# YyzHarry/imbalanced-regression

Measured on NVIDIA H100. Metric: images/sec, higher is better.
Workload: dtype bf16

## Files before the change

imbalanced-regression_b200/_convlib.py:

```python
from ctypes import c_float, c_int, c_int64, c_size_t, c_void_p

import _lib

P = c_void_p
_I9 = [c_int] * 9

_lib.register({
    "dirb200_conv_prep_weights": (c_int, [P, c_int, c_int, c_int, c_int, c_int, P, P, P]),
    "dirb200_input_to_s2d": (c_int, [P, c_int, c_int, c_int, P, P]),
    "dirb200_conv_fprop": (c_int, [P, P, P] + _I9 + [c_int, P]),
    "dirb200_conv_dgrad": (c_int, [P, P, P] + _I9 + [P]),
    "dirb200_conv_wgrad_workspace_bytes": (c_size_t, _I9 + [c_int]),
    "dirb200_conv_wgrad": (c_int, [P, P, P, P, c_size_t] + _I9 + [c_int, c_int, P]),
    "dirb200_conv_plan": (c_int, _I9 + [c_int, c_int, P]),
    "dirb200_conv_fprop_upsampled": (c_int, [P, P, P] + [c_int] * 7 + [P]),
    "dirb200_conv_wgrad_upsampled_workspace_bytes": (c_size_t, [c_int] * 7),
    "dirb200_conv_wgrad_upsampled": (c_int, [P, P, P, P, c_size_t] + [c_int] * 8 + [P]),
    "dirb200_bn_eval_coeffs": (c_int, [c_int, P, P, c_float, P, P, P, P, P]),
    "dirb200_conv_fprop_bn_stats": (c_int, [P, P, P] + _I9 + [c_int, P, P, P]),
    "dirb200_conv_fprop_affine": (c_int, [P, P, P] + _I9 + [P, P, P, c_int, P]),
    "dirb200_conv_dgrad_bn_moments": (c_int, [P, P, P] + _I9 + [P, P, P, P, P, P]),
    "dirb200_bn_finalize_layout": (c_int, [P, P, c_int64, c_int, P, P, c_float, c_float, P, P, P, P, P, P, P]),
    "dirb200_bn_bwd_coeffs_layout": (c_int, [P, P, c_int64, c_int, P, P, P, P, P, P, P]),
})
```

imbalanced-regression_b200/csrc/conv.cuh:

```cuda
#pragma once
#include "common.cuh"

namespace dirb200 {

struct ConvShape {
  int n, h, w, cin, cout, kh, kw, stride, pad, ho, wo;
};

struct StatLayout {
  int rows, n_tiles, bn, group;
};

int conv_fprop(const __nv_bfloat16* x, const __nv_bfloat16* w, __nv_bfloat16* y, const ConvShape& s, bool stem,
               cudaStream_t st, float* stat_partial = nullptr, StatLayout* layout = nullptr);
struct ConvEpilogue {
  const float* scale;
  const float* shift;
  const __nv_bfloat16* residual;
  bool relu;
};
int conv_fprop_affine(const __nv_bfloat16* x, const __nv_bfloat16* w, __nv_bfloat16* out, const ConvShape& s,
                      const ConvEpilogue& epi, cudaStream_t st);
struct DgradBnMoments {
  const __nv_bfloat16* y;
  const float *scale, *shift;
  float* partial;
  StatLayout* layout;
};
bool conv_dgrad_fuses_bn_moments(const ConvShape& s);
int conv_dgrad(const __nv_bfloat16* dy, const __nv_bfloat16* wt, __nv_bfloat16* dx, const ConvShape& s,
               cudaStream_t st, const DgradBnMoments* bnm = nullptr);
int conv_wgrad_splits(const ConvShape& s);
size_t conv_wgrad_workspace_bytes(const ConvShape& s);
int conv_wgrad_partials(const __nv_bfloat16* x, const __nv_bfloat16* dy, float* partial, const ConvShape& s, bool stem,
                        int* splits_out, cudaStream_t st);
int wgrad_reduce(const float* workspace, int splits, float* dw, const ConvShape& s, bool stem, bool accumulate,
                 cudaStream_t st);
int check_upsampled_conv(int n, int h, int w, int cin, int cout, int ho, int wo, const char* who);
int conv_fprop_upsampled(const __nv_bfloat16* x, const __nv_bfloat16* w_fprop, __nv_bfloat16* y, int n, int h, int w,
                         int cin, int cout, int ho, int wo, cudaStream_t st);
size_t conv_wgrad_upsampled_workspace_bytes(int n, int cin, int cout, int ho, int wo);
int conv_wgrad_partials_upsampled(const __nv_bfloat16* x, const __nv_bfloat16* dy, float* partial, int n, int h, int w,
                                  int cin, int cout, int ho, int wo, int* splits_out, cudaStream_t st);
int conv_wgrad(const __nv_bfloat16* x, const __nv_bfloat16* dy, float* dw, float* workspace, const ConvShape& s,
               bool stem, bool accumulate, cudaStream_t st);
struct WgradReduceDesc {
  const float* partial;
  size_t w_off;
  int splits, cout, cin, kh, kw, stem;
};
int wgrad_reduce_all(const WgradReduceDesc* descs_dev, int nlayers, float* grads, cudaStream_t st);
struct PrepDesc {
  size_t w_off;
  int cout, cin, kh, kw, stem;
  __nv_bfloat16 *wf, *wd;
  FastDiv fd_cin, fd_cout, fd_taps;
};
inline PrepDesc make_prep_desc(size_t w_off, int cout, int cin, int kh, int kw, int stem, __nv_bfloat16* wf,
                               __nv_bfloat16* wd) {
  PrepDesc d{w_off, cout, cin, kh, kw, stem, wf, wd, {}, {}, {}};
  d.fd_cin = make_fastdiv((uint32_t)cin);
  d.fd_cout = make_fastdiv((uint32_t)cout);
  d.fd_taps = make_fastdiv((uint32_t)(kh * kw));
  return d;
}
int conv_plan(const ConvShape& s, bool stem, int op, int* plan);
int prep_weights_all(const float* params, const PrepDesc* descs_dev, int nlayers, cudaStream_t st);
int prep_weights(const float* w, int cout, int cin, int kh, int kw, bool stem, __nv_bfloat16* wf, __nv_bfloat16* wd,
                 cudaStream_t st);
int input_to_s2d(const float* x, int n, int h, int w, __nv_bfloat16* out, cudaStream_t st);

}
```

imbalanced-regression_b200/csrc/conv_api.cu:

```cuda
#include "common.cuh"
#include "conv.cuh"

namespace dirb200 {

__global__ void prep_weights_kernel(const float* __restrict__ w, int cout, int cin, int kh, int kw,
                                    __nv_bfloat16* __restrict__ wf, __nv_bfloat16* __restrict__ wd) {
  const int64_t total = (int64_t)cout * cin * kh * kw;
  for (int64_t i = blockIdx.x * (int64_t)blockDim.x + threadIdx.x; i < total; i += (int64_t)gridDim.x * blockDim.x) {
    int c = (int)(i % cin);
    int64_t t = i / cin;
    int s = (int)(t % kw); t /= kw;
    int r = (int)(t % kh);
    int co = (int)(t / kh);
    const float v = w[(((int64_t)co * cin + c) * kh + r) * kw + s];
    const __nv_bfloat16 b = __float2bfloat16_rn(v);
    wf[i] = b;
    if (wd) wd[(((int64_t)c * kh + r) * kw + s) * cout + co] = b;
  }
}

__global__ void prep_stem_weights_kernel(const float* __restrict__ w, int cout, __nv_bfloat16* __restrict__ wf) {
  const int total = cout * 256;
  for (int i = blockIdx.x * blockDim.x + threadIdx.x; i < total; i += gridDim.x * blockDim.x) {
    const int co = i >> 8, k = i & 255;
    const int rp = k >> 6, sp = (k >> 4) & 3, ph = (k >> 3) & 1, pw = (k >> 2) & 1, c = k & 3;
    const int r = 2 * rp + ph - 1, s = 2 * sp + pw - 1;
    float v = 0.f;
    if (c < 3 && r >= 0 && s >= 0 && r < 7 && s < 7) v = w[((co * 3 + c) * 7 + r) * 7 + s];
    wf[i] = __float2bfloat16_rn(v);
  }
}

__global__ void input_to_s2d_kernel(const float* __restrict__ x, int n, int h, int w, __nv_bfloat16* __restrict__ out) {
  const int h2 = h / 2, w2 = w / 2;
  const int64_t total = (int64_t)n * h2 * w2;
  for (int64_t i = blockIdx.x * (int64_t)blockDim.x + threadIdx.x; i < total; i += (int64_t)gridDim.x * blockDim.x) {
    const int xw = (int)(i % w2);
    const int yh = (int)((i / w2) % h2);
    const int b = (int)(i / ((int64_t)w2 * h2));
    __align__(16) __nv_bfloat16 v[16];
#pragma unroll
    for (int ph = 0; ph < 2; ++ph)
#pragma unroll
      for (int pw = 0; pw < 2; ++pw) {
#pragma unroll
        for (int c = 0; c < 3; ++c)
          v[(ph * 2 + pw) * 4 + c] =
              __float2bfloat16_rn(x[(((int64_t)b * 3 + c) * h + (2 * yh + ph)) * w + (2 * xw + pw)]);
        v[(ph * 2 + pw) * 4 + 3] = __float2bfloat16_rn(0.f);
      }
    uint4* o = reinterpret_cast<uint4*>(out + i * 16);
    o[0] = reinterpret_cast<uint4*>(v)[0];
    o[1] = reinterpret_cast<uint4*>(v)[1];
  }
}

__global__ void wgrad_reduce_kernel(const float* __restrict__ partial, int splits, int cout, int cin, int kh, int kw,
                                    int accumulate, float* __restrict__ dw) {
  const int64_t ktot = (int64_t)kh * kw * cin;
  const int64_t total = ktot * cout;
  const int64_t i = blockIdx.x * (int64_t)blockDim.x + threadIdx.x;
  if (i >= total) return;
  const int co = (int)(i / ktot);
  const int64_t k = i - (int64_t)co * ktot;
  float acc = 0.f;
  for (int sp = 0; sp < splits; ++sp) acc += partial[(int64_t)sp * total + i];
  const int c = (int)(k % cin);
  const int t = (int)(k / cin);
  float* o = dw + ((int64_t)co * cin + c) * (kh * kw) + t;
  *o = accumulate ? *o + acc : acc;
}

__global__ void wgrad_reduce_stem_kernel(const float* __restrict__ partial, int splits, int cout, int accumulate,
                                         float* __restrict__ dw) {
  const int total = 256 * cout;
  for (int i = blockIdx.x * blockDim.x + threadIdx.x; i < total; i += gridDim.x * blockDim.x) {
    const int co = i >> 8, k = i & 255;
    const int rp = k >> 6, sp_ = (k >> 4) & 3, ph = (k >> 3) & 1, pw = (k >> 2) & 1, c = k & 3;
    const int r = 2 * rp + ph - 1, s = 2 * sp_ + pw - 1;
    if (c >= 3 || r < 0 || s < 0) continue;
    float acc = 0.f;
    for (int sp = 0; sp < splits; ++sp) acc += partial[(int64_t)sp * total + i];
    float* o = dw + ((co * 3 + c) * 7 + r) * 7 + s;
    *o = accumulate ? *o + acc : acc;
  }
}

__global__ void __launch_bounds__(256)
wgrad_reduce_all_kernel(const WgradReduceDesc* __restrict__ descs, float* __restrict__ grads) {
  const WgradReduceDesc d = descs[blockIdx.y];
  float* dw = grads + d.w_off;
  if (d.stem) {
    const int total = 256 * d.cout;
    for (int i = blockIdx.x * blockDim.x + threadIdx.x; i < total; i += gridDim.x * blockDim.x) {
      const int co = i >> 8, k = i & 255;
      const int rp = k >> 6, sp_ = (k >> 4) & 3, ph = (k >> 3) & 1, pw = (k >> 2) & 1, c = k & 3;
      const int r = 2 * rp + ph - 1, s = 2 * sp_ + pw - 1;
      if (c >= 3 || r < 0 || s < 0) continue;
      float acc = 0.f;
      for (int sp = 0; sp < d.splits; ++sp) acc += d.partial[(int64_t)sp * total + i];
      dw[((co * 3 + c) * 7 + r) * 7 + s] += acc;
    }
    return;
  }
  const int64_t ktot = (int64_t)d.kh * d.kw * d.cin;
  const int64_t total = ktot * d.cout;
  const int taps = d.kh * d.kw;
  for (int64_t i = blockIdx.x * (int64_t)blockDim.x + threadIdx.x; i < total; i += (int64_t)gridDim.x * blockDim.x) {
    const float* p = d.partial + i;
    float a0 = 0.f, a1 = 0.f, a2 = 0.f, a3 = 0.f;
    int sp = 0;
    for (; sp + 4 <= d.splits; sp += 4) {
      a0 += p[(int64_t)sp * total];
      a1 += p[(int64_t)(sp + 1) * total];
      a2 += p[(int64_t)(sp + 2) * total];
      a3 += p[(int64_t)(sp + 3) * total];
    }
    for (; sp < d.splits; ++sp) a0 += p[(int64_t)sp * total];
    const int64_t co = i / ktot, k = i - co * ktot;
    const int c = (int)(k % d.cin), t = (int)(k / d.cin);
    dw[(co * d.cin + c) * taps + t] += (a0 + a1) + (a2 + a3);
  }
}

int wgrad_reduce_all(const WgradReduceDesc* descs_dev, int nlayers, float* grads, cudaStream_t st) {
  if (nlayers <= 0) return DIRB200_OK;
  wgrad_reduce_all_kernel<<<dim3(2 * num_sms(), nlayers), 256, 0, st>>>(descs_dev, grads);
  DIRB_LAUNCHED();
  return DIRB200_OK;
}

__global__ void prep_weights_all_kernel(const float* __restrict__ params, const PrepDesc* __restrict__ descs) {
  const PrepDesc d = descs[blockIdx.y];
  const float* w = params + d.w_off;
  if (d.stem) {
    const int total = d.cout * 256;
    for (int i = blockIdx.x * blockDim.x + threadIdx.x; i < total; i += gridDim.x * blockDim.x) {
      const int co = i >> 8, k = i & 255;
      const int rp = k >> 6, sp = (k >> 4) & 3, ph = (k >> 3) & 1, pw = (k >> 2) & 1, c = k & 3;
      const int r = 2 * rp + ph - 1, s = 2 * sp + pw - 1;
      float v = 0.f;
      if (c < 3 && r >= 0 && s >= 0 && r < 7 && s < 7) v = w[((co * 3 + c) * 7 + r) * 7 + s];
      d.wf[i] = __float2bfloat16_rn(v);
    }
    return;
  }
  const uint32_t taps = (uint32_t)(d.kh * d.kw);
  const uint32_t total = (uint32_t)d.cout * (uint32_t)d.cin * taps;
  const uint32_t stride = gridDim.x * blockDim.x;
  for (uint32_t i = blockIdx.x * blockDim.x + threadIdx.x; i < total; i += stride) {
    uint32_t t, c, co, tap;
    d.fd_cin.divmod(i, t, c);
    d.fd_taps.divmod(t, co, tap);
    d.wf[i] = __float2bfloat16_rn(w[((size_t)co * d.cin + c) * taps + tap]);
  }
  if (!d.wd) return;
  for (uint32_t i = blockIdx.x * blockDim.x + threadIdx.x; i < total; i += stride) {
    uint32_t t, c, co, tap;
    d.fd_cout.divmod(i, t, co);
    d.fd_taps.divmod(t, c, tap);
    d.wd[i] = __float2bfloat16_rn(w[((size_t)co * d.cin + c) * taps + tap]);
  }
}

int prep_weights_all(const float* params, const PrepDesc* descs_dev, int nlayers, cudaStream_t st) {
  prep_weights_all_kernel<<<dim3(96, nlayers), 256, 0, st>>>(params, descs_dev);
  DIRB_LAUNCHED();
  return DIRB200_OK;
}

static inline int grid1d(int64_t n, int block = 256) {
  int64_t g = (n + block - 1) / block;
  const int64_t cap = 8 * (int64_t)num_sms();
  return (int)(g < 1 ? 1 : (g > cap ? cap : g));
}

int prep_weights(const float* w, int cout, int cin, int kh, int kw, bool stem, __nv_bfloat16* wf, __nv_bfloat16* wd,
                 cudaStream_t st) {
  if (stem) {
    prep_stem_weights_kernel<<<grid1d((int64_t)cout * 256), 256, 0, st>>>(w, cout, wf);
  } else {
    prep_weights_kernel<<<grid1d((int64_t)cout * cin * kh * kw), 256, 0, st>>>(w, cout, cin, kh, kw, wf, wd);
  }
  DIRB_LAUNCHED();
  return DIRB200_OK;
}

int input_to_s2d(const float* x, int n, int h, int w, __nv_bfloat16* out, cudaStream_t st) {
  input_to_s2d_kernel<<<grid1d((int64_t)n * (h / 2) * (w / 2)), 256, 0, st>>>(x, n, h, w, out);
  DIRB_LAUNCHED();
  return DIRB200_OK;
}

int wgrad_reduce(const float* workspace, int splits, float* dw, const ConvShape& s, bool stem, bool accumulate,
                 cudaStream_t st) {
  if (stem)
    wgrad_reduce_stem_kernel<<<grid1d(256 * (int64_t)s.cout), 256, 0, st>>>(workspace, splits, s.cout, accumulate, dw);
  else
  {
    const int64_t total = (int64_t)s.kh * s.kw * s.cin * s.cout;
    wgrad_reduce_kernel<<<(unsigned)((total + 255) / 256), 256, 0, st>>>(workspace, splits, s.cout, s.cin, s.kh, s.kw,
                                                                         accumulate, dw);
  }
  DIRB_LAUNCHED();
  return DIRB200_OK;
}

int conv_wgrad(const __nv_bfloat16* x, const __nv_bfloat16* dy, float* dw, float* workspace, const ConvShape& s,
               bool stem, bool accumulate, cudaStream_t st) {
  int splits = 1;
  if (int rc = conv_wgrad_partials(x, dy, workspace, s, stem, &splits, st)) return rc;
  return wgrad_reduce(workspace, splits, dw, s, stem, accumulate, st);
}

static int to_shape(int n, int h, int w, int cin, int cout, int kh, int kw, int stride, int pad, int stem,
                    ConvShape* s) {
  if (stem) {
    DIRB_CHECK_ARG(cin == 3 && kh == 7 && kw == 7 && stride == 2 && pad == 3 && h % 2 == 0 && w % 2 == 0,
                   "stem conv must be 3->Cout 7x7 stride 2 pad 3 on even H, W");
    *s = ConvShape{n, h / 2, w / 2, 16, cout, 4, 4, 1, 2, h / 2, w / 2};
  } else {
    DIRB_CHECK_ARG(n > 0 && h > 0 && w > 0 && kh > 0 && kw > 0 && stride > 0 && pad >= 0, "bad conv shape");
    *s = ConvShape{n, h, w, cin, cout, kh, kw, stride, pad, (h + 2 * pad - kh) / stride + 1,
                   (w + 2 * pad - kw) / stride + 1};
  }
  return DIRB200_OK;
}

}

using namespace dirb200;

extern "C" {

int dirb200_conv_prep_weights(const float* w, int cout, int cin, int kh, int kw, int stem, void* w_fprop,
                              void* w_dgrad, void* stream) {
  DIRB_CHECK_ARG(w && w_fprop && cout > 0 && cin > 0, "conv_prep_weights: bad arguments");
  DIRB_CHECK_ARG(!stem || (cin == 3 && kh == 7 && kw == 7), "conv_prep_weights: stem must be 3x7x7");
  return prep_weights(w, cout, cin, kh, kw, stem != 0, (__nv_bfloat16*)w_fprop, (__nv_bfloat16*)w_dgrad,
                      as_stream(stream));
}

int dirb200_input_to_s2d(const float* x_nchw, int n, int h, int w, void* out_bf16, void* stream) {
  DIRB_CHECK_ARG(x_nchw && out_bf16 && n > 0 && h > 0 && w > 0 && h % 2 == 0 && w % 2 == 0,
                 "input_to_s2d: bad arguments");
  return input_to_s2d(x_nchw, n, h, w, (__nv_bfloat16*)out_bf16, as_stream(stream));
}

int dirb200_conv_fprop(const void* x, const void* w_fprop, void* y, int n, int h, int w, int cin, int cout, int kh,
                       int kw, int stride, int pad, int stem, void* stream) {
  DIRB_CHECK_ARG(x && w_fprop && y, "conv_fprop: null pointer");
  ConvShape s;
  if (int rc = to_shape(n, h, w, cin, cout, kh, kw, stride, pad, stem, &s)) return rc;
  return conv_fprop((const __nv_bfloat16*)x, (const __nv_bfloat16*)w_fprop, (__nv_bfloat16*)y, s, stem != 0,
                    as_stream(stream));
}

int dirb200_conv_dgrad(const void* dy, const void* w_dgrad, void* dx, int n, int h, int w, int cin, int cout, int kh,
                       int kw, int stride, int pad, void* stream) {
  DIRB_CHECK_ARG(dy && w_dgrad && dx, "conv_dgrad: null pointer");
  ConvShape s;
  if (int rc = to_shape(n, h, w, cin, cout, kh, kw, stride, pad, 0, &s)) return rc;
  return conv_dgrad((const __nv_bfloat16*)dy, (const __nv_bfloat16*)w_dgrad, (__nv_bfloat16*)dx, s,
                    as_stream(stream));
}

size_t dirb200_conv_wgrad_workspace_bytes(int n, int h, int w, int cin, int cout, int kh, int kw, int stride, int pad,
                                          int stem) {
  ConvShape s;
  if (to_shape(n, h, w, cin, cout, kh, kw, stride, pad, stem, &s)) return 0;
  return conv_wgrad_workspace_bytes(s);
}

int dirb200_conv_wgrad(const void* x, const void* dy, float* dw, void* workspace, size_t workspace_bytes, int n, int h,
                       int w, int cin, int cout, int kh, int kw, int stride, int pad, int stem, int accumulate,
                       void* stream) {
  DIRB_CHECK_ARG(x && dy && dw && workspace, "conv_wgrad: null pointer");
  ConvShape s;
  if (int rc = to_shape(n, h, w, cin, cout, kh, kw, stride, pad, stem, &s)) return rc;
  if (workspace_bytes < conv_wgrad_workspace_bytes(s)) {
    set_error("conv_wgrad: workspace too small (%zu < %zu)", workspace_bytes, conv_wgrad_workspace_bytes(s));
    return DIRB200_ERR_WORKSPACE;
  }
  return conv_wgrad((const __nv_bfloat16*)x, (const __nv_bfloat16*)dy, dw, (float*)workspace, s, stem != 0,
                    accumulate != 0, as_stream(stream));
}

int dirb200_conv_fprop_upsampled(const void* x, const void* w_fprop, void* y, int n, int h, int w, int cin, int cout,
                                 int ho, int wo, void* stream) {
  DIRB_CHECK_ARG(x && w_fprop && y, "conv_fprop_upsampled: null pointer");
  return conv_fprop_upsampled((const __nv_bfloat16*)x, (const __nv_bfloat16*)w_fprop, (__nv_bfloat16*)y, n, h, w, cin,
                              cout, ho, wo, as_stream(stream));
}

size_t dirb200_conv_wgrad_upsampled_workspace_bytes(int n, int h, int w, int cin, int cout, int ho, int wo) {
  if (check_upsampled_conv(n, h, w, cin, cout, ho, wo, "conv_wgrad_upsampled_workspace_bytes")) return 0;
  return conv_wgrad_upsampled_workspace_bytes(n, cin, cout, ho, wo);
}

int dirb200_conv_wgrad_upsampled(const void* x, const void* dy, float* dw, void* workspace, size_t workspace_bytes, int n,
                                 int h, int w, int cin, int cout, int ho, int wo, int accumulate, void* stream) {
  DIRB_CHECK_ARG(x && dy && dw && workspace, "conv_wgrad_upsampled: null pointer");
  if (int rc = check_upsampled_conv(n, h, w, cin, cout, ho, wo, "conv_wgrad_upsampled")) return rc;
  const size_t need = conv_wgrad_upsampled_workspace_bytes(n, cin, cout, ho, wo);
  if (workspace_bytes < need) {
    set_error("conv_wgrad_upsampled: workspace too small (%zu < %zu)", workspace_bytes, need);
    return DIRB200_ERR_WORKSPACE;
  }
  cudaStream_t st = as_stream(stream);
  int splits = 1;
  if (int rc = conv_wgrad_partials_upsampled((const __nv_bfloat16*)x, (const __nv_bfloat16*)dy, (float*)workspace, n, h,
                                             w, cin, cout, ho, wo, &splits, st))
    return rc;
  const ConvShape s{n, ho, wo, cin, cout, 5, 5, 1, 2, ho, wo};
  return wgrad_reduce((const float*)workspace, splits, dw, s, false, accumulate != 0, st);
}

static void layout_to_host(const StatLayout& l, int* layout_host) {
  layout_host[0] = l.rows; layout_host[1] = l.n_tiles; layout_host[2] = l.bn; layout_host[3] = l.group;
}

int dirb200_conv_fprop_bn_stats(const void* x, const void* w_fprop, void* y, int n, int h, int w, int cin, int cout,
                                int kh, int kw, int stride, int pad, int stem, float* partial, int* layout_host,
                                void* stream) {
  DIRB_CHECK_ARG(x && w_fprop && y && partial && layout_host, "conv_fprop_bn_stats: null pointer");
  ConvShape s;
  if (int rc = to_shape(n, h, w, cin, cout, kh, kw, stride, pad, stem, &s)) return rc;
  StatLayout lay{};
  if (int rc = conv_fprop((const __nv_bfloat16*)x, (const __nv_bfloat16*)w_fprop, (__nv_bfloat16*)y, s, stem != 0,
                          as_stream(stream), partial, &lay))
    return rc;
  layout_to_host(lay, layout_host);
  return DIRB200_OK;
}

int dirb200_conv_fprop_affine(const void* x, const void* w_fprop, void* out, int n, int h, int w, int cin, int cout,
                              int kh, int kw, int stride, int pad, const float* scale, const float* shift,
                              const void* residual, int relu, void* stream) {
  DIRB_CHECK_ARG(x && w_fprop && out, "conv_fprop_affine: null pointer");
  ConvShape s;
  if (int rc = to_shape(n, h, w, cin, cout, kh, kw, stride, pad, 0, &s)) return rc;
  return conv_fprop_affine((const __nv_bfloat16*)x, (const __nv_bfloat16*)w_fprop, (__nv_bfloat16*)out, s,
                           ConvEpilogue{scale, shift, (const __nv_bfloat16*)residual, relu != 0}, as_stream(stream));
}

int dirb200_conv_dgrad_bn_moments(const void* dy, const void* w_dgrad, void* dx, int n, int h, int w, int cin, int cout,
                                  int kh, int kw, int stride, int pad, const void* y_prev, const float* scale,
                                  const float* shift, float* partial, int* layout_host, void* stream) {
  DIRB_CHECK_ARG(dy && w_dgrad && dx && y_prev && scale && shift && partial && layout_host,
                 "conv_dgrad_bn_moments: null pointer");
  ConvShape s;
  if (int rc = to_shape(n, h, w, cin, cout, kh, kw, stride, pad, 0, &s)) return rc;
  StatLayout lay{};
  const DgradBnMoments bm{(const __nv_bfloat16*)y_prev, scale, shift, partial, &lay};
  if (int rc = conv_dgrad((const __nv_bfloat16*)dy, (const __nv_bfloat16*)w_dgrad, (__nv_bfloat16*)dx, s,
                          as_stream(stream), &bm))
    return rc;
  layout_to_host(lay, layout_host);
  return DIRB200_OK;
}

int dirb200_conv_plan(int n, int h, int w, int cin, int cout, int kh, int kw, int stride, int pad, int stem, int op,
                      int* plan7) {
  DIRB_CHECK_ARG(plan7 && op >= 0 && op <= 2, "conv_plan: bad arguments");
  ConvShape s;
  if (int rc = to_shape(n, h, w, cin, cout, kh, kw, stride, pad, stem, &s)) return rc;
  return conv_plan(s, stem != 0, op, plan7);
}

}
```

imbalanced-regression_b200/csrc/conv_igemm.cu:

```cuda
#include <stdlib.h>
#include "common.cuh"
#include "tc.cuh"
#include "conv.cuh"
#include "upsample.cuh"

namespace dirb200 {
using namespace tc;

constexpr int BM = 128;
constexpr int BK = 64;
constexpr int kProducerThreads = 128;
constexpr int kThreads = 384;
constexpr int kMaxTaps = 25;
constexpr int kMaxSmemBytes = 232448;

struct IgemmParams {
  const __nv_bfloat16* src;
  int n, hs, ws, cs;
  int hm, wm;
  int kh, kw, stride, pad;
  int transposed;
  int cls_on, cls_py, cls_px, full_h, full_w;
  int ntaps_c;
  int tap_list[kMaxTaps];
  long long tap_eoff[kMaxTaps];
  unsigned short tap_r[kMaxTaps], tap_s[kMaxTaps];
  FastDiv fd_hw, fd_wm, fd_cpb, fd_kw, fd_ntiles, fd_persplit;
  int cpb;
  long long pixels;
  int num_kblocks;
  int kblocks_per_split;
  int total_chunks;
  int m_tiles, n_tiles;
  int num_tiles;
  int a_mode;
  int i2c_stride, i2c_lo;
  int ldc;
  void* out;
  float* stat_out;
  const float* epi_scale;
  const float* epi_shift;
  const __nv_bfloat16* epi_res;
  int epi_relu;
  const __nv_bfloat16* bst_y;
  const float* bst_scale;
  const float* bst_shift;
  int up_h, up_w;
  float up_sh, up_sw;
};

template <int BN, bool STAGED_EPI>
struct Cfg {
  static constexpr int kABytes = BM * BK * 2;
  static constexpr int kBBytes = BN * BK * 2;
  static constexpr int kStageBytes = kABytes + kBBytes;
  static constexpr int kStages = BN == 128 ? (STAGED_EPI ? 5 : 6) : 8;
  static constexpr int kBarOffset = kStages * kStageBytes;
  static constexpr int kStageRowBytes = BN * 2 + 16;
  static constexpr int kEpiWarpBytes = 16 * kStageRowBytes;
  static constexpr int kEpiOffset = kBarOffset + 256;
  static constexpr int kStatWarpBytes = 2 * BN * 4;
  static constexpr int kStatOffset = kEpiOffset + (STAGED_EPI ? 8 * kEpiWarpBytes : 0);
  static constexpr int kSmemBytes = kStatOffset + (STAGED_EPI ? 8 * kStatWarpBytes : 0) + 1024;
  static_assert(kSmemBytes <= kMaxSmemBytes, "shared memory budget");
};

__device__ __forceinline__ uint32_t pack_pixel(long long p, const IgemmParams& P) {
  if (p >= P.pixels) return 0u;
  uint32_t n, rem, y, x;
  P.fd_hw.divmod(static_cast<uint32_t>(p), n, rem);
  P.fd_wm.divmod(rem, y, x);
  return 0x80000000u | (n << 18) | (y << 9) | x;
}

struct RowPre {
  int nb, yb, xb;
};
__device__ __forceinline__ RowPre row_pre(const IgemmParams& P, uint32_t pk) {
  RowPre rp;
  const int n = (pk >> 18) & 0x1FFF;
  int y = (pk >> 9) & 0x1FF, x = pk & 0x1FF;
  if (P.cls_on) {
    y = 2 * y + P.cls_py;
    x = 2 * x + P.cls_px;
  }
  rp.nb = n * P.hs;
  if (!P.transposed) {
    rp.yb = y * P.stride - P.pad;
    rp.xb = x * P.stride - P.pad;
  } else {
    rp.yb = y + P.pad;
    rp.xb = x + P.pad;
  }
  if (!(pk >> 31)) rp.yb = -(1 << 28);
  return rp;
}

__device__ __forceinline__ const __nv_bfloat16* tap_source(const IgemmParams& P, const RowPre& rp, int r, int s,
                                                           int coff, bool& ok) {
  int hi, wi;
  ok = true;
  if (!P.transposed) {
    hi = rp.yb + r;
    wi = rp.xb + s;
  } else {
    hi = rp.yb - r;
    wi = rp.xb - s;
    if (P.stride == 2) {
      ok = ((hi | wi) & 1) == 0;
      hi >>= 1;
      wi >>= 1;
    }
  }
  ok = ok && static_cast<unsigned>(hi) < static_cast<unsigned>(P.hs) &&
       static_cast<unsigned>(wi) < static_cast<unsigned>(P.ws);
  return ok ? P.src + (static_cast<size_t>(rp.nb + hi) * P.ws + wi) * P.cs + coff : P.src;
}

__device__ __forceinline__ uint4 upsampled_16b(const IgemmParams& P, uint32_t pk, int r, int s, int coff) {
  const int n = (pk >> 18) & 0x1FFF;
  const int uy = static_cast<int>((pk >> 9) & 0x1FF) - P.pad + r, ux = static_cast<int>(pk & 0x1FF) - P.pad + s;
  uint4 out = make_uint4(0u, 0u, 0u, 0u);
  if ((pk >> 31) && static_cast<unsigned>(uy) < static_cast<unsigned>(P.hs) &&
      static_cast<unsigned>(ux) < static_cast<unsigned>(P.ws)) {
    int y0, y1, x0, x1;
    float ly, lx;
    upsample_src_index(uy, P.up_sh, P.up_h, y0, y1, ly);
    upsample_src_index(ux, P.up_sw, P.up_w, x0, x1, lx);
    const __nv_bfloat16* base = P.src + static_cast<size_t>(n) * P.up_h * P.up_w * P.cs + coff;
    const uint4 a00 = __ldg(reinterpret_cast<const uint4*>(base + (static_cast<size_t>(y0) * P.up_w + x0) * P.cs));
    const uint4 a01 = __ldg(reinterpret_cast<const uint4*>(base + (static_cast<size_t>(y0) * P.up_w + x1) * P.cs));
    const uint4 a10 = __ldg(reinterpret_cast<const uint4*>(base + (static_cast<size_t>(y1) * P.up_w + x0) * P.cs));
    const uint4 a11 = __ldg(reinterpret_cast<const uint4*>(base + (static_cast<size_t>(y1) * P.up_w + x1) * P.cs));
    const float hy = __fsub_rn(1.f, ly), hx = __fsub_rn(1.f, lx);
    const uint32_t w00[4] = {a00.x, a00.y, a00.z, a00.w}, w01[4] = {a01.x, a01.y, a01.z, a01.w};
    const uint32_t w10[4] = {a10.x, a10.y, a10.z, a10.w}, w11[4] = {a11.x, a11.y, a11.z, a11.w};
    uint32_t o[4];
#pragma unroll
    for (int e = 0; e < 4; ++e) {
      const float lo = upsample_lerp(__uint_as_float(w00[e] << 16), __uint_as_float(w01[e] << 16),
                                     __uint_as_float(w10[e] << 16), __uint_as_float(w11[e] << 16), hx, lx, hy, ly);
      const float hi = upsample_lerp(__uint_as_float(w00[e] & 0xffff0000u), __uint_as_float(w01[e] & 0xffff0000u),
                                     __uint_as_float(w10[e] & 0xffff0000u), __uint_as_float(w11[e] & 0xffff0000u), hx,
                                     lx, hy, ly);
      __nv_bfloat162 h = __floats2bfloat162_rn(lo, hi);
      o[e] = *reinterpret_cast<uint32_t*>(&h);
    }
    out = make_uint4(o[0], o[1], o[2], o[3]);
  }
  return out;
}
template <int BN, bool WGRAD, bool STEM, bool ATMA = false, bool AFFINE = false, bool BSTAT = false, bool UPS = false>
__global__ void __launch_bounds__(kThreads, 1)
igemm_kernel(const __grid_constant__ CUtensorMap tmap_b, const __grid_constant__ CUtensorMap tmap_a,
             const IgemmParams P) {
  using C = Cfg<BN, !WGRAD>;
  static_assert(BN == 64 || BN == 128, "tile width: one m64n64 / m64n128 wgmma per warpgroup and k step");
  static_assert(!ATMA || !STEM, "TMA-fed A operand: not for the stem");
  static_assert(!AFFINE || (!WGRAD && !STEM), "folded-BN epilogue: non-stem fprop GEMMs only");
  static_assert(!BSTAT || (ATMA && !WGRAD && !AFFINE), "BN-backward moments in the epilogue: TMA-fed dgrad GEMMs only");
  static_assert(!UPS || (!ATMA && !STEM && !AFFINE && !BSTAT), "up-sampled A operand: plain fprop / wgrad GEMMs only");
  extern __shared__ uint8_t smem_raw[];
  const uint32_t smem_base = (smem_u32(smem_raw) + 1023u) & ~1023u;
  uint8_t* const smem_gen = smem_raw + (smem_base - smem_u32(smem_raw));
  const uint32_t bar_base = smem_base + C::kBarOffset;
  auto a_addr = [&](int s) { return smem_base + s * C::kStageBytes; };
  auto b_addr = [&](int s) { return smem_base + s * C::kStageBytes + C::kABytes; };
  constexpr uint32_t nstages = C::kStages;
  auto full_bar = [&](int s) { return bar_base + 8u * s; };
  auto empty_bar = [&](int s) { return bar_base + 8u * (C::kStages + s); };
  const int warp = static_cast<int>(threadIdx.x >> 5), lane = threadIdx.x & 31;

  int tile_first, tile_end, tile_step, fixed_n = 0;
  if constexpr (WGRAD) {
    tile_first = blockIdx.x; tile_end = P.num_tiles; tile_step = gridDim.x;
  } else {
    uint32_t gi, nn;
    P.fd_ntiles.divmod(blockIdx.x, gi, nn);
    fixed_n = static_cast<int>(nn);
    tile_first = static_cast<int>(gi);
    tile_end = P.m_tiles;
    tile_step = static_cast<int>(P.fd_ntiles.div(gridDim.x - 1u - nn)) + 1;
  }
  auto decode_tile = [&](int t, int& split, int& m_tile, int& n_tile, int& kb_begin, int& nk) {
    if constexpr (WGRAD) {
      uint32_t sp, rem, mt, nt;
      P.fd_persplit.divmod(static_cast<uint32_t>(t), sp, rem);
      P.fd_ntiles.divmod(rem, mt, nt);
      split = static_cast<int>(sp);
      m_tile = static_cast<int>(mt);
      n_tile = static_cast<int>(nt);
      kb_begin = split * P.kblocks_per_split;
      const int kb_end = min(P.num_kblocks, kb_begin + P.kblocks_per_split);
      nk = max(0, kb_end - kb_begin);
    } else {
      split = 0;
      m_tile = t;
      n_tile = fixed_n;
      kb_begin = 0;
      nk = P.num_kblocks;
    }
  };

  if (threadIdx.x == 0) {
    for (int s = 0; s < C::kStages; ++s) {
      mbar_init(full_bar(s), ATMA ? 1 : kProducerThreads + 1);
      mbar_init(empty_bar(s), 8);
    }
    fence_barrier_init();
  }
  __syncthreads();

  if (warp < 4) {
    if constexpr (UPS) {
      const int j = lane & 7;
      const int q = lane >> 3;
      uint32_t rs = 0, rph = 0;
      for (int t = tile_first; t < tile_end; t += tile_step) {
        int split, m_tile, n_tile, kb_begin, nk;
        decode_tile(t, split, m_tile, n_tile, kb_begin, nk);
        const int n0 = n_tile * BN;
        uint32_t pk8[8];
        int chunk_r = 0, chunk_s = 0, chunk_c0 = 0;
        bool chunk_ok = true;
        uint32_t tile_off;
        if constexpr (!WGRAD) {
          const uint32_t mypk = pack_pixel(static_cast<long long>(m_tile) * BM + warp * 32 + lane, P);
#pragma unroll
          for (int i = 0; i < 8; ++i) pk8[i] = __shfl_sync(0xffffffffu, mypk, 4 * i + q);
          tile_off = warp * 32 * 128;
        } else {
          const int chunk = warp >> 1;
          const int gchunk = m_tile * 2 + chunk;
          chunk_ok = gchunk < P.total_chunks;
          uint32_t tap, cbk, cr, csx;
          P.fd_cpb.divmod(static_cast<uint32_t>(gchunk), tap, cbk);
          P.fd_kw.divmod(tap, cr, csx);
          chunk_c0 = static_cast<int>(cbk) * 64;
          chunk_r = static_cast<int>(cr);
          chunk_s = static_cast<int>(csx);
          tile_off = chunk * 8192 + (warp & 1) * 32 * 128;
        }
        int tc = 0, cb = 0;
        for (int it = 0; it < nk; ++it) {
          const int s = static_cast<int>(rs);
          mbar_wait(empty_bar(s), rph ^ 1u);
          if (++rs == nstages) { rs = 0; rph ^= 1u; }
          const int kb = kb_begin + it;
          const uint32_t dst_base = a_addr(s) + tile_off;
          int kcoord = kb, r, sx, coff;
          uint32_t mypk = 0u;
          if constexpr (!WGRAD) {
            r = P.tap_r[tc];
            sx = P.tap_s[tc];
            coff = cb * 64 + j * 8;
            kcoord = P.tap_list[tc] * P.cpb + cb;
            if (++cb == P.cpb) { cb = 0; ++tc; }
          } else {
            r = chunk_r;
            sx = chunk_s;
            coff = chunk_c0 + j * 8;
            mypk = chunk_ok ? pack_pixel(static_cast<long long>(kb) * 64 + (warp & 1) * 32 + lane, P) : 0u;
          }
#pragma unroll
          for (int i = 0; i < 8; ++i) {
            const int row = 4 * i + q;
            const uint32_t pk = WGRAD ? __shfl_sync(0xffffffffu, mypk, row) : pk8[i];
            const uint4 v = upsampled_16b(P, pk, r, sx, coff);
            asm volatile("st.shared.v4.b32 [%0], {%1, %2, %3, %4};" ::"r"(dst_base + row * 128 + ((j ^ (row & 7)) << 4)),
                         "r"(v.x), "r"(v.y), "r"(v.z), "r"(v.w) : "memory");
          }
          if (warp == 0) {
            if (elect_one()) {
              mbar_arrive_expect_tx(full_bar(s), C::kBBytes);
              if constexpr (!WGRAD) {
                tma_load_2d(b_addr(s), &tmap_b, full_bar(s), kcoord * BK, n0);
              } else {
#pragma unroll
                for (int i = 0; i < BN / 64; ++i)
                  tma_load_2d(b_addr(s) + i * 8192, &tmap_b, full_bar(s), n0 + 64 * i, kb * 64);
              }
            }
            __syncwarp();
          }
          fence_proxy_async();
          mbar_arrive(full_bar(s));
        }
      }
    } else if constexpr (!ATMA) {
      const int j = lane & 7;
      const int q = lane >> 3;
      uint32_t rs = 0, rph = 0;
      for (int t = tile_first; t < tile_end; t += tile_step) {
        int split, m_tile, n_tile, kb_begin, nk;
        decode_tile(t, split, m_tile, n_tile, kb_begin, nk);
        const int n0 = n_tile * BN;
        long long off8[8];
        uint32_t mask8[8];
        int chunk_r = 0, chunk_s = 0, chunk_c0 = 0;
        bool chunk_ok = true;
        uint32_t tile_off = 0;
        if constexpr (!WGRAD) {
          const RowPre rp = row_pre(P, pack_pixel(static_cast<long long>(m_tile) * BM + warp * 32 + lane, P));
          const bool rvalid = rp.yb > -(1 << 27);
          int oy = rp.yb, ox = rp.xb;
          if (P.transposed && P.stride == 2) { oy >>= 1; ox >>= 1; }
          const long long my_off = (static_cast<long long>(rp.nb + oy) * P.ws + ox) * P.cs;
          uint32_t vy = 0, vx = 0;
          if (rvalid) {
            const int nky = P.kh, nkx = STEM ? 4 : P.kw;
            for (int r = 0; r < nky; ++r) {
              int h = P.transposed ? rp.yb - r : rp.yb + r;
              bool ok = true;
              if (P.transposed && P.stride == 2) { ok = (h & 1) == 0; h >>= 1; }
              vy |= (ok && static_cast<unsigned>(h) < static_cast<unsigned>(P.hs) ? 1u : 0u) << r;
            }
            for (int c = 0; c < nkx; ++c) {
              int w = P.transposed ? rp.xb - c : rp.xb + c;
              bool ok = true;
              if (P.transposed && P.stride == 2) { ok = (w & 1) == 0; w >>= 1; }
              vx |= (ok && static_cast<unsigned>(w) < static_cast<unsigned>(P.ws) ? 1u : 0u) << c;
            }
          }
          uint32_t my_mask;
          if constexpr (STEM) {
            my_mask = vy | (vx << 8);
          } else {
            my_mask = 0;
            for (int r = 0; r < P.kh; ++r)
              if ((vy >> r) & 1u) my_mask |= vx << (r * P.kw);
          }
#pragma unroll
          for (int i = 0; i < 8; ++i) {
            const int row = 4 * i + q;
            const long long o = __shfl_sync(0xffffffffu, my_off, row);
            const uint32_t m = __shfl_sync(0xffffffffu, my_mask, row);
            if constexpr (STEM) {
              off8[i] = o + (j >> 1) * P.cs + (j & 1) * 8;
              mask8[i] = ((m >> (8 + (j >> 1))) & 1u) ? (m & 0xFu) : 0u;
            } else {
              off8[i] = o + j * 8;
              mask8[i] = m;
            }
          }
          tile_off = warp * 32 * 128;
        } else {
          const int chunk = warp >> 1;
          const int gchunk = m_tile * 2 + chunk;
          chunk_ok = gchunk < P.total_chunks;
          if constexpr (STEM) {
            chunk_r = gchunk;
          } else {
            uint32_t tap, cb, cr, csx;
            P.fd_cpb.divmod(static_cast<uint32_t>(gchunk), tap, cb);
            P.fd_kw.divmod(tap, cr, csx);
            chunk_c0 = static_cast<int>(cb) * 64;
            chunk_r = static_cast<int>(cr);
            chunk_s = static_cast<int>(csx);
          }
          tile_off = chunk * 8192 + (warp & 1) * 32 * 128;
        }
        int tc = 0, cb = 0;
        long long stem_toff = 0;
        for (int it = 0; it < nk; ++it) {
          const int s = static_cast<int>(rs);
          mbar_wait(empty_bar(s), rph ^ 1u);
          if (++rs == nstages) { rs = 0; rph ^= 1u; }
          const int kb = kb_begin + it;
          const uint32_t dst_base = a_addr(s) + tile_off;
          int kcoord = kb;
          if constexpr (!WGRAD) {
            int tp;
            long long toff;
            if constexpr (STEM) {
              tp = kb;
              toff = stem_toff;
              stem_toff += static_cast<long long>(P.ws) * P.cs;
            } else {
              tp = P.tap_list[tc];
              toff = P.tap_eoff[tc] + cb * 64;
              kcoord = tp * P.cpb + cb;
              if (++cb == P.cpb) { cb = 0; ++tc; }
            }
#pragma unroll
            for (int i = 0; i < 8; ++i) {
              const int row = 4 * i + q;
              const bool ok = (mask8[i] >> tp) & 1u;
              const __nv_bfloat16* src = ok ? P.src + (off8[i] + toff) : P.src;
              cp_async16(dst_base + row * 128 + ((j ^ (row & 7)) << 4), src, ok ? 16u : 0u);
            }
          } else {
            const uint32_t mypk = chunk_ok ? pack_pixel(static_cast<long long>(kb) * 64 + (warp & 1) * 32 + lane, P) : 0u;
            const RowPre rp = row_pre(P, mypk);
            bool myok;
            const __nv_bfloat16* myptr = tap_source(P, rp, chunk_r, STEM ? 0 : chunk_s, STEM ? 0 : chunk_c0, myok);
            const unsigned long long myaddr = reinterpret_cast<unsigned long long>(myptr);
            uint32_t okbits;
            if constexpr (STEM) {
              okbits = 0;
              const bool rowok = (mypk >> 31) && static_cast<unsigned>(rp.yb + chunk_r) < static_cast<unsigned>(P.hs);
              for (int sp = 0; sp < 4; ++sp)
                okbits |= (rowok && static_cast<unsigned>(rp.xb + sp) < static_cast<unsigned>(P.ws) ? 1u : 0u) << sp;
            } else {
              okbits = myok ? 1u : 0u;
            }
            unsigned long long rowaddr = myaddr;
            if constexpr (STEM)
              rowaddr = reinterpret_cast<unsigned long long>(
                  P.src + ((static_cast<long long>(rp.nb + rp.yb + chunk_r) * P.ws + rp.xb) * P.cs));
#pragma unroll
            for (int i = 0; i < 8; ++i) {
              const int row = 4 * i + q;
              const unsigned long long a = __shfl_sync(0xffffffffu, rowaddr, row);
              const uint32_t okb = __shfl_sync(0xffffffffu, okbits, row);
              const bool ok = STEM ? ((okb >> (j >> 1)) & 1u) : (okb & 1u);
              const __nv_bfloat16* src = reinterpret_cast<const __nv_bfloat16*>(a) + j * 8;
              cp_async16(dst_base + row * 128 + ((j ^ (row & 7)) << 4), ok ? src : P.src, ok ? 16u : 0u);
            }
          }
          if (warp == 0) {
            if (elect_one()) {
              mbar_arrive_expect_tx(full_bar(s), C::kBBytes);
              if constexpr (!WGRAD) {
                tma_load_2d(b_addr(s), &tmap_b, full_bar(s), kcoord * BK, n0);
              } else {
#pragma unroll
                for (int i = 0; i < BN / 64; ++i)
                  tma_load_2d(b_addr(s) + i * 8192, &tmap_b, full_bar(s), n0 + 64 * i, kb * 64);
              }
            }
            __syncwarp();
          }
          cp_async_mbar_arrive_noinc(full_bar(s));
        }
      }
    } else if (warp == 0) {
      uint32_t rs = 0, rph = 0;
      for (int t = tile_first; t < tile_end; t += tile_step) {
        int split, m_tile, n_tile, kb_begin, nk;
        decode_tile(t, split, m_tile, n_tile, kb_begin, nk);
        const int n0 = n_tile * BN;
        int tile_w0 = 0, tile_h0 = 0, tile_n0 = 0;
        if constexpr (!WGRAD) {
          if (P.a_mode == 2) {
            uint32_t tn, rem, y0, x0;
            P.fd_hw.divmod(static_cast<uint32_t>(m_tile) * BM, tn, rem);
            P.fd_wm.divmod(rem, y0, x0);
            tile_n0 = static_cast<int>(tn);
            tile_w0 = static_cast<int>(x0) * P.i2c_stride + P.i2c_lo;
            tile_h0 = static_cast<int>(y0) * P.i2c_stride + P.i2c_lo;
          }
        }
        int tc = 0, cb = 0;
        for (int it = 0; it < nk; ++it) {
          const int s = static_cast<int>(rs);
          mbar_wait(empty_bar(s), rph ^ 1u);
          if (++rs == nstages) { rs = 0; rph ^= 1u; }
          const int kb = kb_begin + it;
          if (elect_one()) {
            if constexpr (!WGRAD) {
              mbar_arrive_expect_tx(full_bar(s), C::kBBytes + C::kABytes);
              if (P.a_mode == 1)
                tma_load_2d(a_addr(s), &tmap_a, full_bar(s), kb * BK, m_tile * BM);
              else
                tma_load_im2col_4d(a_addr(s), &tmap_a, full_bar(s), cb * BK, tile_w0, tile_h0, tile_n0,
                                   P.tap_s[tc], P.tap_r[tc]);
              tma_load_2d(b_addr(s), &tmap_b, full_bar(s), (P.tap_list[tc] * P.cpb + cb) * BK, n0);
            } else {
              const int nchunks = min(2, P.total_chunks - 2 * m_tile);
              mbar_arrive_expect_tx(full_bar(s), C::kBBytes + nchunks * 8192);
              if (P.a_mode == 1) {
                for (int i = 0; i < nchunks; ++i)
                  tma_load_2d(a_addr(s) + i * 8192, &tmap_a, full_bar(s), (2 * m_tile + i) * 64, kb * 64);
              } else {
                uint32_t n0i, rem, y0, x0;
                P.fd_hw.divmod(static_cast<uint32_t>(kb) * 64u, n0i, rem);
                P.fd_wm.divmod(rem, y0, x0);
                for (int i = 0; i < nchunks; ++i) {
                  uint32_t tap, cbk, r, sx;
                  P.fd_cpb.divmod(static_cast<uint32_t>(2 * m_tile + i), tap, cbk);
                  P.fd_kw.divmod(tap, r, sx);
                  tma_load_im2col_4d(a_addr(s) + i * 8192, &tmap_a, full_bar(s), static_cast<int>(cbk) * 64,
                                     static_cast<int>(x0) * P.i2c_stride + P.i2c_lo,
                                     static_cast<int>(y0) * P.i2c_stride + P.i2c_lo, static_cast<int>(n0i),
                                     static_cast<uint16_t>(sx), static_cast<uint16_t>(r));
                }
              }
#pragma unroll
              for (int i = 0; i < BN / 64; ++i)
                tma_load_2d(b_addr(s) + i * 8192, &tmap_b, full_bar(s), n0 + 64 * i, kb * 64);
            }
          }
          if constexpr (!WGRAD) {
            if (++cb == P.cpb) { cb = 0; ++tc; }
          }
          __syncwarp();
        }
      }
    }
    return;
  }

  const int g = (warp >> 2) - 1;
  const int wq = warp & 3;
  const int ew = g * 4 + wq;
  const int fr = lane >> 2, fc = 2 * (lane & 3);
  float* const stat_sm = reinterpret_cast<float*>(smem_gen + C::kStatOffset) + ew * (2 * BN);
  if constexpr (!WGRAD) {
    if (P.stat_out != nullptr)
      for (int i = lane; i < 2 * BN; i += 32) stat_sm[i] = 0.f;
  }
  constexpr uint32_t kLbo = WGRAD ? 8192u : 16u;
  constexpr uint32_t kadv = WGRAD ? (2048u >> 4) : (32u >> 4);
  constexpr int kT = WGRAD ? 1 : 0;
  float acc[BN / 2];
  uint32_t rs = 0, rph = 0;
  for (int t = tile_first; t < tile_end; t += tile_step) {
    int split, m_tile, n_tile, kb_begin, nk;
    decode_tile(t, split, m_tile, n_tile, kb_begin, nk);
    int prev = 0;
    for (int it = 0; it < nk; ++it) {
      const int s = static_cast<int>(rs);
      mbar_wait(full_bar(s), rph);
      if (++rs == nstages) { rs = 0; rph ^= 1u; }
      if constexpr (!ATMA) fence_proxy_async();
      const uint64_t adesc = make_smem_desc(a_addr(s) + g * 8192, kLbo, 1024u);
      const uint64_t bdesc = make_smem_desc(b_addr(s), kLbo, 1024u);
      wgmma_fence_operands(acc);
      wgmma_fence();
#pragma unroll
      for (int k = 0; k < BK / 16; ++k)
        wgmma_bf16<BN, kT, kT>(acc, adesc + static_cast<uint64_t>(k * kadv), bdesc + static_cast<uint64_t>(k * kadv),
                               (it > 0 || k > 0) ? 1u : 0u);
      wgmma_commit();
      wgmma_fence_operands(acc);
      if (it > 0) {
        wgmma_wait<1>();
        if (lane == 0) mbar_arrive(empty_bar(prev));
      }
      prev = s;
    }
    wgmma_wait<0>();
    wgmma_fence_operands(acc);
    if (nk > 0 && lane == 0) mbar_arrive(empty_bar(prev));
    const int n0 = n_tile * BN;

    if constexpr (!WGRAD) {
      const uint32_t stage_base = smem_base + C::kEpiOffset + ew * C::kEpiWarpBytes;
      const bool relu_now = AFFINE && P.epi_relu && P.epi_res == nullptr;
#pragma unroll
      for (int j = 0; j < BN / 8; ++j) {
        const int col = 8 * j + fc;
        float v0 = acc[4 * j], v1 = acc[4 * j + 1], v2 = acc[4 * j + 2], v3 = acc[4 * j + 3];
        if constexpr (AFFINE) {
          const float2 a = __ldg(reinterpret_cast<const float2*>(P.epi_scale + n0 + col));
          const float2 b = __ldg(reinterpret_cast<const float2*>(P.epi_shift + n0 + col));
          v0 = fmaf(v0, a.x, b.x); v1 = fmaf(v1, a.y, b.y); v2 = fmaf(v2, a.x, b.x); v3 = fmaf(v3, a.y, b.y);
          if (relu_now) { v0 = fmaxf(v0, 0.f); v1 = fmaxf(v1, 0.f); v2 = fmaxf(v2, 0.f); v3 = fmaxf(v3, 0.f); }
        }
        __nv_bfloat162 h0 = __floats2bfloat162_rn(v0, v1), h1 = __floats2bfloat162_rn(v2, v3);
        asm volatile("st.shared.b32 [%0], %1;" ::"r"(stage_base + fr * C::kStageRowBytes + col * 2),
                     "r"(*reinterpret_cast<uint32_t*>(&h0)) : "memory");
        asm volatile("st.shared.b32 [%0], %1;" ::"r"(stage_base + (fr + 8) * C::kStageRowBytes + col * 2),
                     "r"(*reinterpret_cast<uint32_t*>(&h1)) : "memory");
      }
      __syncwarp();
      constexpr int kLanesPerRow = BN * 2 / 16;
      constexpr int kRowsPerIter = 32 / kLanesPerRow;
      constexpr int kIters = 16 / kRowsPerIter;
      const int sub = lane / kLanesPerRow, col16 = lane % kLanesPerRow;
      const long long p0 = static_cast<long long>(m_tile) * BM + g * 64 + wq * 16;
      __nv_bfloat16* out_cols = reinterpret_cast<__nv_bfloat16*>(P.out) + n0 + col16 * 8;
#pragma unroll
      for (int i = 0; i < kIters; ++i) {
        const int rl = i * kRowsPerIter + sub;
        const long long p = p0 + rl;
        int orow = (p < P.pixels && nk > 0) ? static_cast<int>(p) : -1;
        if (orow >= 0 && P.cls_on) {
          const uint32_t pk = pack_pixel(p, P);
          const int n = (pk >> 18) & 0x1FFF, yy = (pk >> 9) & 0x1FF, xx = pk & 0x1FF;
          orow = (n * P.full_h + 2 * yy + P.cls_py) * P.full_w + 2 * xx + P.cls_px;
        }
        if (orow >= 0) {
          uint4 val;
          asm volatile("ld.shared.v4.b32 {%0, %1, %2, %3}, [%4];"
                       : "=r"(val.x), "=r"(val.y), "=r"(val.z), "=r"(val.w)
                       : "r"(stage_base + rl * C::kStageRowBytes + col16 * 16));
          if constexpr (AFFINE) {
            if (P.epi_res != nullptr) {
              const uint4 rv = *reinterpret_cast<const uint4*>(P.epi_res + n0 + col16 * 8 + static_cast<long long>(orow) * P.ldc);
              uint32_t o[4] = {val.x, val.y, val.z, val.w};
              const uint32_t rr[4] = {rv.x, rv.y, rv.z, rv.w};
#pragma unroll
              for (int e = 0; e < 4; ++e) {
                float lo = __uint_as_float(o[e] << 16) + __uint_as_float(rr[e] << 16);
                float hi = __uint_as_float(o[e] & 0xffff0000u) + __uint_as_float(rr[e] & 0xffff0000u);
                if (P.epi_relu) { lo = fmaxf(lo, 0.f); hi = fmaxf(hi, 0.f); }
                __nv_bfloat162 h = __floats2bfloat162_rn(lo, hi);
                o[e] = *reinterpret_cast<uint32_t*>(&h);
              }
              val = make_uint4(o[0], o[1], o[2], o[3]);
            }
          }
          *reinterpret_cast<uint4*>(out_cols + static_cast<long long>(orow) * P.ldc) = val;
        }
      }
      if (BSTAT || P.stat_out != nullptr) {
#pragma unroll
        for (int h = 0; h < BN / 64; ++h) {
          const int col = 2 * (lane + 32 * h);
          float s0 = 0.f, s1 = 0.f, q0 = 0.f, q1 = 0.f;
          float2 bsc = make_float2(0.f, 0.f), bsh = bsc;
          if constexpr (BSTAT) {
            bsc = __ldg(reinterpret_cast<const float2*>(P.bst_scale + n0 + col));
            bsh = __ldg(reinterpret_cast<const float2*>(P.bst_shift + n0 + col));
          }
#pragma unroll
          for (int r = 0; r < 16; ++r) {
            uint32_t w;
            asm volatile("ld.shared.b32 %0, [%1];" : "=r"(w) : "r"(stage_base + r * C::kStageRowBytes + col * 2));
            float g0 = __uint_as_float(w << 16), g1 = __uint_as_float(w & 0xffff0000u);
            if constexpr (BSTAT) {
              const long long p = p0 + r;
              const uint32_t yw = p < P.pixels ? __ldg(reinterpret_cast<const unsigned int*>(P.bst_y + p * P.ldc + n0 + col)) : 0u;
              const float y0 = __uint_as_float(yw << 16), y1 = __uint_as_float(yw & 0xffff0000u);
              if (!(fmaf(y0, bsc.x, bsh.x) > 0.f)) g0 = 0.f;
              if (!(fmaf(y1, bsc.y, bsh.y) > 0.f)) g1 = 0.f;
              s0 += g0; s1 += g1;
              q0 = fmaf(g0, y0, q0); q1 = fmaf(g1, y1, q1);
            } else {
              s0 += g0; s1 += g1;
              q0 = fmaf(g0, g0, q0); q1 = fmaf(g1, g1, q1);
            }
          }
          stat_sm[col] += s0;
          stat_sm[col + 1] += s1;
          stat_sm[BN + col] += q0;
          stat_sm[BN + col + 1] += q1;
        }
      }
      __syncwarp();
    } else {
      const int ktot = P.total_chunks * 64;
      const int krow = m_tile * BM + g * 64 + wq * 16 + fr;
      float* out = reinterpret_cast<float*>(P.out) + (static_cast<size_t>(split) * P.ldc + n0) * ktot;
#pragma unroll
      for (int j = 0; j < BN / 8; ++j) {
        const size_t c0 = static_cast<size_t>(8 * j + fc) * ktot;
#pragma unroll
        for (int e = 0; e < 2; ++e) {
          if (krow < ktot) out[c0 + e * ktot + krow] = nk > 0 ? acc[4 * j + e] : 0.f;
          if (krow + 8 < ktot) out[c0 + e * ktot + krow + 8] = nk > 0 ? acc[4 * j + 2 + e] : 0.f;
        }
      }
    }
  }
  if constexpr (!WGRAD) {
    if (P.stat_out != nullptr) {
      asm volatile("bar.sync 1, 256;" ::: "memory");
      const float* all = reinterpret_cast<const float*>(smem_gen + C::kStatOffset);
      float* dst = P.stat_out + static_cast<size_t>(blockIdx.x) * 2 * P.ldc + fixed_n * BN;
      for (int o = static_cast<int>(threadIdx.x) - kProducerThreads; o < 2 * BN; o += kThreads - kProducerThreads) {
        const int k = o / BN, col = o - k * BN;
        const float v = ((all[o] + all[2 * BN + o]) + (all[4 * BN + o] + all[6 * BN + o])) +
                        ((all[8 * BN + o] + all[10 * BN + o]) + (all[12 * BN + o] + all[14 * BN + o]));
        dst[static_cast<size_t>(k) * P.ldc + col] = v;
      }
    }
  }
}

typedef CUresult (*EncodeTiledFn)(CUtensorMap*, CUtensorMapDataType, cuuint32_t, void*, const cuuint64_t*,
                                  const cuuint64_t*, const cuuint32_t*, const cuuint32_t*, CUtensorMapInterleave,
                                  CUtensorMapSwizzle, CUtensorMapL2promotion, CUtensorMapFloatOOBfill);

static EncodeTiledFn encode_fn() {
  static EncodeTiledFn fn = nullptr;
  if (!fn) {
    void* p = nullptr;
    cudaDriverEntryPointQueryResult q;
    if (cudaGetDriverEntryPoint("cuTensorMapEncodeTiled", &p, cudaEnableDefault, &q) == cudaSuccess &&
        q == cudaDriverEntryPointSuccess)
      fn = reinterpret_cast<EncodeTiledFn>(p);
  }
  return fn;
}

int make_tmap_bf16_2d(CUtensorMap* tm, const void* ptr, uint64_t inner, uint64_t outer, uint64_t row_stride_bytes,
                      uint32_t box_outer) {
  EncodeTiledFn fn = encode_fn();
  if (!fn) {
    set_error("cuTensorMapEncodeTiled entry point not available");
    return DIRB200_ERR_CUDA;
  }
  cuuint64_t dims[2] = {inner, outer};
  cuuint64_t strides[1] = {row_stride_bytes};
  cuuint32_t box[2] = {64, box_outer};
  cuuint32_t estr[2] = {1, 1};
  CUresult r = fn(tm, CU_TENSOR_MAP_DATA_TYPE_BFLOAT16, 2, const_cast<void*>(ptr), dims, strides, box, estr,
                  CU_TENSOR_MAP_INTERLEAVE_NONE, CU_TENSOR_MAP_SWIZZLE_128B, CU_TENSOR_MAP_L2_PROMOTION_L2_256B,
                  CU_TENSOR_MAP_FLOAT_OOB_FILL_NONE);
  if (r != CUDA_SUCCESS) {
    set_error("cuTensorMapEncodeTiled failed (%d) inner=%llu outer=%llu stride=%llu", (int)r,
              (unsigned long long)inner, (unsigned long long)outer, (unsigned long long)row_stride_bytes);
    return DIRB200_ERR_CUDA;
  }
  return DIRB200_OK;
}

typedef CUresult (*EncodeIm2colFn)(CUtensorMap*, CUtensorMapDataType, cuuint32_t, void*, const cuuint64_t*,
                                   const cuuint64_t*, const int*, const int*, cuuint32_t, cuuint32_t, const cuuint32_t*,
                                   CUtensorMapInterleave, CUtensorMapSwizzle, CUtensorMapL2promotion,
                                   CUtensorMapFloatOOBfill);
int make_tmap_im2col_bf16(CUtensorMap* tm, const void* ptr, int c, int w, int h, int n, int lower_w, int lower_h,
                          int upper_w, int upper_h, int trav, int pixels_per_col) {
  static EncodeIm2colFn fn = nullptr;
  if (!fn) {
    void* p = nullptr;
    cudaDriverEntryPointQueryResult q;
    if (cudaGetDriverEntryPoint("cuTensorMapEncodeIm2col", &p, cudaEnableDefault, &q) == cudaSuccess &&
        q == cudaDriverEntryPointSuccess)
      fn = reinterpret_cast<EncodeIm2colFn>(p);
  }
  if (!fn) {
    set_error("cuTensorMapEncodeIm2col entry point not available");
    return DIRB200_ERR_CUDA;
  }
  cuuint64_t dims[4] = {(cuuint64_t)c, (cuuint64_t)w, (cuuint64_t)h, (cuuint64_t)n};
  cuuint64_t strides[3] = {(cuuint64_t)c * 2, (cuuint64_t)w * c * 2, (cuuint64_t)h * w * c * 2};
  int lower[2] = {lower_w, lower_h}, upper[2] = {upper_w, upper_h};
  cuuint32_t estr[4] = {1, (cuuint32_t)trav, (cuuint32_t)trav, 1};
  CUresult r = fn(tm, CU_TENSOR_MAP_DATA_TYPE_BFLOAT16, 4, const_cast<void*>(ptr), dims, strides, lower, upper, 64,
                  (cuuint32_t)pixels_per_col, estr, CU_TENSOR_MAP_INTERLEAVE_NONE, CU_TENSOR_MAP_SWIZZLE_128B,
                  CU_TENSOR_MAP_L2_PROMOTION_L2_256B, CU_TENSOR_MAP_FLOAT_OOB_FILL_NONE);
  if (r != CUDA_SUCCESS) {
    set_error("cuTensorMapEncodeIm2col failed (%d) c=%d w=%d h=%d n=%d lower=%d,%d upper=%d,%d stride=%d", (int)r, c, w, h,
              n, lower_w, lower_h, upper_w, upper_h, trav);
    return DIRB200_ERR_CUDA;
  }
  int drv = 0;
  if (cudaDriverGetVersion(&drv) == cudaSuccess && drv <= 13010 && (size_t)c * w * h * n * 2 < 131072)
    reinterpret_cast<uint64_t*>(tm)[1] &= ~(1ull << 21);
  return DIRB200_OK;
}
static thread_local StatLayout t_last_layout{};

static IgemmParams finish_params(const IgemmParams& P) {
  IgemmParams Q = P;
  Q.fd_hw = make_fastdiv(static_cast<uint32_t>(Q.hm * Q.wm));
  Q.fd_wm = make_fastdiv(static_cast<uint32_t>(Q.wm));
  Q.fd_cpb = make_fastdiv(static_cast<uint32_t>(Q.cpb > 0 ? Q.cpb : 1));
  Q.fd_kw = make_fastdiv(static_cast<uint32_t>(Q.kw > 0 ? Q.kw : 1));
  Q.fd_ntiles = make_fastdiv(static_cast<uint32_t>(Q.n_tiles > 0 ? Q.n_tiles : 1));
  Q.fd_persplit = make_fastdiv(static_cast<uint32_t>(Q.m_tiles * Q.n_tiles > 0 ? Q.m_tiles * Q.n_tiles : 1));
  const int nt = Q.ntaps_c < kMaxTaps ? Q.ntaps_c : kMaxTaps;
  for (int i = 0; i < kMaxTaps; ++i) {
    Q.tap_eoff[i] = 0;
    Q.tap_r[i] = Q.tap_s[i] = 0;
  }
  for (int i = 0; i < nt && Q.kw > 0; ++i) {
    const int tp = Q.tap_list[i];
    int r = tp / Q.kw, sx = tp - r * Q.kw;
    if (Q.transposed && Q.cls_on) {
      Q.tap_r[i] = static_cast<unsigned short>((Q.cls_py + Q.pad - r) / 2 - Q.i2c_lo);
      Q.tap_s[i] = static_cast<unsigned short>((Q.cls_px + Q.pad - sx) / 2 - Q.i2c_lo);
      r >>= 1; sx >>= 1;
      Q.tap_eoff[i] = -static_cast<long long>(r * Q.ws + sx) * Q.cs;
    } else if (Q.transposed) {
      Q.tap_r[i] = static_cast<unsigned short>(Q.kh - 1 - r);
      Q.tap_s[i] = static_cast<unsigned short>(Q.kw - 1 - sx);
      if (Q.stride == 2) { r >>= 1; sx >>= 1; }
      Q.tap_eoff[i] = -static_cast<long long>(r * Q.ws + sx) * Q.cs;
    } else {
      Q.tap_r[i] = static_cast<unsigned short>(r);
      Q.tap_s[i] = static_cast<unsigned short>(sx);
      Q.tap_eoff[i] = static_cast<long long>(r * Q.ws + sx) * Q.cs;
    }
  }
  return Q;
}

template <int BN, bool WGRAD, bool STEM, bool ATMA = false, bool AFFINE = false, bool BSTAT = false, bool UPS = false>
static int launch_igemm_impl(const CUtensorMap& tm, const CUtensorMap& tma, const IgemmParams& Qin, cudaStream_t st) {
  using C = Cfg<BN, !WGRAD>;
  const IgemmParams Q = finish_params(Qin);
  static bool configured = false;
  if (!configured) {
    DIRB_CUDA(cudaFuncSetAttribute(igemm_kernel<BN, WGRAD, STEM, ATMA, AFFINE, BSTAT, UPS>,
                                   cudaFuncAttributeMaxDynamicSharedMemorySize, C::kSmemBytes));
    configured = true;
  }
  int grid = Q.num_tiles < num_sms() ? Q.num_tiles : num_sms();
  if (!WGRAD && grid < Q.n_tiles) grid = Q.n_tiles;
  t_last_layout = StatLayout{grid, Q.n_tiles, BN, 1};
  igemm_kernel<BN, WGRAD, STEM, ATMA, AFFINE, BSTAT, UPS><<<grid, kThreads, C::kSmemBytes, st>>>(tm, tma, Q);
  DIRB_LAUNCHED();
  return DIRB200_OK;
}

template <int BN, bool WGRAD, bool STEM>
static int launch_igemm(const CUtensorMap& tm, const IgemmParams& P, int m_tiles, int splits, cudaStream_t st,
                        const CUtensorMap* tma = nullptr) {
  IgemmParams Q = P;
  Q.m_tiles = m_tiles;
  Q.num_tiles = m_tiles * P.n_tiles * splits;
  if constexpr (!STEM) {
    if (tma) {
      if constexpr (!WGRAD) {
        if (Q.epi_scale != nullptr) return launch_igemm_impl<BN, false, false, true, true>(tm, *tma, Q, st);
        if (Q.bst_y != nullptr) return launch_igemm_impl<BN, false, false, true, false, true>(tm, *tma, Q, st);
      }
      return launch_igemm_impl<BN, WGRAD, false, true>(tm, *tma, Q, st);
    }
  }
  if constexpr (!WGRAD && !STEM) {
    if (Q.epi_scale != nullptr) return launch_igemm_impl<BN, false, false, false, true>(tm, tm, Q, st);
  }
  if (Q.epi_scale != nullptr || Q.bst_y != nullptr) {
    set_error("conv: the BN-backward moments epilogue needs a TMA-fed A operand; the folded-BN one a non-stem fprop");
    return DIRB200_ERR_ARG;
  }
  return launch_igemm_impl<BN, WGRAD, STEM>(tm, tm, Q, st);
}

static int pick_bn(int n_dim) { return n_dim % 128 == 0 ? 128 : 64; }

#define DISPATCH_BN(bn, WG, ST, ...) \
  ((bn) == 128 ? launch_igemm<128, WG, ST>(__VA_ARGS__) : launch_igemm<64, WG, ST>(__VA_ARGS__))

static int check_shape(const ConvShape& s, bool stem, const char* who) {
  DIRB_CHECK_ARG(s.n > 0 && s.h > 0 && s.w > 0 && s.kh > 0 && s.kw > 0 && s.stride > 0 && s.pad >= 0,
                 "%s: bad conv shape", who);
  DIRB_CHECK_ARG(s.cout % 64 == 0, "%s: Cout must be a multiple of 64 (got %d)", who, s.cout);
  DIRB_CHECK_ARG(static_cast<long long>(s.n) * s.h * s.w < (1LL << 31) && static_cast<long long>(s.n) * s.ho * s.wo < (1LL << 31),
                 "%s: more than 2^31 pixels", who);
  if (stem)
    DIRB_CHECK_ARG(s.cin == 16 && s.kh == 4 && s.kw == 4 && s.stride == 1, "%s: stem expects the 4x4x16 s2d form", who);
  else
    DIRB_CHECK_ARG(s.cin % 64 == 0, "%s: Cin must be a multiple of 64 (got %d)", who, s.cin);
  return DIRB200_OK;
}

static bool atma_enabled() {
  static const bool on = [] {
    const char* e = getenv("DIRB200_ATMA");
    return !(e != nullptr && e[0] == '0');
  }();
  return on;
}
static bool is_plain_gemm(const ConvShape& s, bool stem) {
  return !stem && s.kh == 1 && s.kw == 1 && s.stride == 1 && s.pad == 0 && atma_enabled();
}
static bool im2col_enabled() {
  static const bool on = [] {
    const char* e = getenv("DIRB200_IM2COL");
    return !(e != nullptr && e[0] == '0');
  }();
  return on && atma_enabled();
}

static int conv_fprop_impl(const __nv_bfloat16* x, const __nv_bfloat16* w, __nv_bfloat16* y, const ConvShape& s, bool stem,
                           cudaStream_t st, float* stat_partial, const ConvEpilogue* epi);

int conv_fprop(const __nv_bfloat16* x, const __nv_bfloat16* w, __nv_bfloat16* y, const ConvShape& s, bool stem,
               cudaStream_t st, float* stat_partial, StatLayout* layout) {
  const int rc = conv_fprop_impl(x, w, y, s, stem, st, stat_partial, nullptr);
  if (layout) *layout = t_last_layout;
  return rc;
}

int conv_fprop_affine(const __nv_bfloat16* x, const __nv_bfloat16* w, __nv_bfloat16* out, const ConvShape& s,
                      const ConvEpilogue& epi, cudaStream_t st) {
  DIRB_CHECK_ARG(epi.scale && epi.shift, "conv_fprop_affine: scale / shift missing");
  return conv_fprop_impl(x, w, out, s, false, st, nullptr, &epi);
}

static int conv_fprop_impl(const __nv_bfloat16* x, const __nv_bfloat16* w, __nv_bfloat16* y, const ConvShape& s, bool stem,
                           cudaStream_t st, float* stat_partial, const ConvEpilogue* epi) {
  if (int rc = check_shape(s, stem, "conv_fprop")) return rc;
  const int ktot = s.kh * s.kw * s.cin;
  IgemmParams P{};
  P.src = x; P.n = s.n; P.hs = s.h; P.ws = s.w; P.cs = s.cin; P.hm = s.ho; P.wm = s.wo;
  P.kh = s.kh; P.kw = s.kw; P.stride = s.stride; P.pad = s.pad; P.transposed = 0;
  P.cpb = stem ? 1 : s.cin / 64;
  P.pixels = static_cast<long long>(s.n) * s.ho * s.wo;
  P.num_kblocks = ktot / 64;
  P.ntaps_c = s.kh * s.kw;
  DIRB_CHECK_ARG(stem || P.ntaps_c <= kMaxTaps, "conv_fprop: at most %d filter taps (got %dx%d)", kMaxTaps, s.kh, s.kw);
  for (int i = 0; i < kMaxTaps; ++i) P.tap_list[i] = i;
  P.ldc = s.cout; P.out = y;
  P.stat_out = stat_partial;
  if (epi) {
    P.epi_scale = epi->scale; P.epi_shift = epi->shift; P.epi_res = epi->residual; P.epi_relu = epi->relu ? 1 : 0;
  }
  const int m_tiles = static_cast<int>((P.pixels + BM - 1) / BM);
  const int bn = pick_bn(s.cout);
  P.n_tiles = s.cout / bn;
  CUtensorMap tm, ta;
  bool tma_fed = false;
  if (is_plain_gemm(s, stem)) {
    if (int rc = make_tmap_bf16_2d(&ta, x, s.cin, static_cast<uint64_t>(P.pixels), static_cast<uint64_t>(s.cin) * 2, BM))
      return rc;
    P.a_mode = 1;
    tma_fed = true;
  } else if (!stem && im2col_enabled()) {
    if (int rc = make_tmap_im2col_bf16(&ta, x, s.cin, s.w, s.h, s.n, -s.pad, -s.pad, s.pad - (s.kw - 1),
                                       s.pad - (s.kh - 1), s.stride, BM))
      return rc;
    P.a_mode = 2; P.i2c_stride = s.stride; P.i2c_lo = -s.pad;
    tma_fed = true;
  }
  if (int rc = make_tmap_bf16_2d(&tm, w, ktot, s.cout, static_cast<uint64_t>(ktot) * 2, bn)) return rc;
  if (stem) return DISPATCH_BN(bn, false, true, tm, P, m_tiles, 1, st);
  if (tma_fed) return DISPATCH_BN(bn, false, false, tm, P, m_tiles, 1, st, &ta);
  return DISPATCH_BN(bn, false, false, tm, P, m_tiles, 1, st);
}

bool conv_dgrad_fuses_bn_moments(const ConvShape& s) {
  return s.stride == 1 && (is_plain_gemm(s, false) || (im2col_enabled() && s.kh == s.kw));
}

int conv_dgrad(const __nv_bfloat16* dy, const __nv_bfloat16* wt, __nv_bfloat16* dx, const ConvShape& s,
               cudaStream_t st, const DgradBnMoments* bnm) {
  if (int rc = check_shape(s, false, "conv_dgrad")) return rc;
  DIRB_CHECK_ARG(!bnm || (conv_dgrad_fuses_bn_moments(s) && bnm->y && bnm->scale && bnm->shift && bnm->partial),
                 "conv_dgrad: BN-backward moments are fused into TMA-fed stride-1 dgrads only");
  DIRB_CHECK_ARG(s.stride == 1 || s.stride == 2, "conv_dgrad: stride must be 1 or 2 (got %d)", s.stride);
  DIRB_CHECK_ARG(s.kh * s.kw <= (s.stride == 1 ? kMaxTaps : 9), "conv_dgrad: at most %d filter taps (stride 2: 9; got %dx%d)",
                 kMaxTaps, s.kh, s.kw);
  const int ktot = s.kh * s.kw * s.cout;
  IgemmParams P{};
  P.src = dy; P.n = s.n; P.hs = s.ho; P.ws = s.wo; P.cs = s.cout; P.hm = s.h; P.wm = s.w;
  P.kh = s.kh; P.kw = s.kw; P.stride = s.stride; P.pad = s.pad; P.transposed = 1;
  P.cpb = s.cout / 64;
  P.ldc = s.cin; P.out = dx;
  if (bnm) {
    P.bst_y = bnm->y; P.bst_scale = bnm->scale; P.bst_shift = bnm->shift; P.stat_out = bnm->partial;
  }
  const int bn = pick_bn(s.cin);
  CUtensorMap tm;
  if (int rc = make_tmap_bf16_2d(&tm, wt, ktot, s.cin, static_cast<uint64_t>(ktot) * 2, bn)) return rc;
  if (s.stride == 1) {
    P.pixels = static_cast<long long>(s.n) * s.h * s.w;
    P.ntaps_c = s.kh * s.kw;
    for (int i = 0; i < kMaxTaps; ++i) P.tap_list[i] = i;
    P.num_kblocks = ktot / 64;
    const int m_tiles = static_cast<int>((P.pixels + BM - 1) / BM);
    P.n_tiles = s.cin / bn;
    CUtensorMap ta;
    bool tma_fed = false;
    if (is_plain_gemm(s, false)) {
      if (int rc = make_tmap_bf16_2d(&ta, dy, s.cout, static_cast<uint64_t>(P.pixels), static_cast<uint64_t>(s.cout) * 2, BM))
        return rc;
      P.a_mode = 1;
      tma_fed = true;
    } else if (im2col_enabled() && s.kh == s.kw) {
      const int lo = s.pad - (s.kh - 1);
      if (int rc = make_tmap_im2col_bf16(&ta, dy, s.cout, s.wo, s.ho, s.n, lo, lo, lo + s.w - s.wo, lo + s.h - s.ho, 1, BM))
        return rc;
      P.a_mode = 2; P.i2c_stride = 1; P.i2c_lo = lo;
      tma_fed = true;
    }
    const int rc = tma_fed ? DISPATCH_BN(bn, false, false, tm, P, m_tiles, 1, st, &ta)
                           : DISPATCH_BN(bn, false, false, tm, P, m_tiles, 1, st);
    if (bnm && bnm->layout) *bnm->layout = t_last_layout;
    return rc;
  }
  bool need_zero = false;
  for (int cls = 0; cls < 4; ++cls) {
    const int py = cls >> 1, px = cls & 1;
    int nt = 0;
    for (int r = 0; r < s.kh; ++r)
      for (int q = 0; q < s.kw; ++q)
        if (((py + s.pad - r) & 1) == 0 && ((px + s.pad - q) & 1) == 0) ++nt;
    if (nt == 0) need_zero = true;
  }
  if (need_zero)
    DIRB_CUDA(cudaMemsetAsync(dx, 0, static_cast<size_t>(s.n) * s.h * s.w * s.cin * sizeof(__nv_bfloat16), st));
  for (int cls = 0; cls < 4; ++cls) {
    IgemmParams Q = P;
    Q.cls_on = 1; Q.cls_py = cls >> 1; Q.cls_px = cls & 1; Q.full_h = s.h; Q.full_w = s.w;
    Q.hm = (s.h - Q.cls_py + 1) / 2;
    Q.wm = (s.w - Q.cls_px + 1) / 2;
    Q.ntaps_c = 0;
    for (int r = 0; r < s.kh; ++r)
      for (int q = 0; q < s.kw; ++q)
        if (((Q.cls_py + s.pad - r) & 1) == 0 && ((Q.cls_px + s.pad - q) & 1) == 0) Q.tap_list[Q.ntaps_c++] = r * s.kw + q;
    if (Q.ntaps_c == 0 || Q.hm <= 0 || Q.wm <= 0) continue;
    Q.pixels = static_cast<long long>(s.n) * Q.hm * Q.wm;
    Q.num_kblocks = Q.ntaps_c * Q.cpb;
    const int m_tiles = static_cast<int>((Q.pixels + BM - 1) / BM);
    Q.n_tiles = s.cin / bn;
    if (im2col_enabled()) {
      int lo = 1 << 20;
      for (int i = 0; i < Q.ntaps_c; ++i) {
        const int r = Q.tap_list[i] / s.kw, q = Q.tap_list[i] % s.kw;
        const int orr = (Q.cls_py + s.pad - r) / 2, oq = (Q.cls_px + s.pad - q) / 2;
        lo = orr < lo ? orr : lo;
        lo = oq < lo ? oq : lo;
      }
      CUtensorMap ta;
      if (int rc = make_tmap_im2col_bf16(&ta, dy, s.cout, s.wo, s.ho, s.n, lo, lo, lo + Q.wm - s.wo, lo + Q.hm - s.ho, 1, BM))
        return rc;
      Q.a_mode = 2; Q.i2c_stride = 1; Q.i2c_lo = lo;
      if (int rc = DISPATCH_BN(bn, false, false, tm, Q, m_tiles, 1, st, &ta)) return rc;
      continue;
    }
    if (int rc = DISPATCH_BN(bn, false, false, tm, Q, m_tiles, 1, st)) return rc;
  }
  return DIRB200_OK;
}

static int wgrad_bn(const ConvShape& s) { return pick_bn(s.cout); }

int conv_wgrad_splits(const ConvShape& s) {
  const long long pixels = static_cast<long long>(s.n) * s.ho * s.wo;
  const int kblocks = static_cast<int>((pixels + 63) / 64);
  const int chunks = s.kh * s.kw * s.cin / 64;
  const int bn = wgrad_bn(s);
  const int m_tiles = (chunks + 1) / 2;
  const int tiles = m_tiles * (s.cout / bn);
  const int sms = num_sms();
  int max_splits = (kblocks + 7) / 8;
  if (max_splits < 1) max_splits = 1;
  int hi = (4 * sms + tiles - 1) / tiles;
  if (hi > max_splits) hi = max_splits;
  int best = 1;
  long long best_cost = -1;
  for (int sp = 1; sp <= hi; ++sp) {
    const long long waves = (static_cast<long long>(tiles) * sp + sms - 1) / sms;
    const long long per = (kblocks + sp - 1) / sp;
    const long long cost = waves * (per + 6);
    if (best_cost < 0 || cost < best_cost) {
      best_cost = cost;
      best = sp;
    }
  }
  return best;
}

size_t conv_wgrad_workspace_bytes(const ConvShape& s) {
  return static_cast<size_t>(conv_wgrad_splits(s)) * s.kh * s.kw * s.cin * s.cout * sizeof(float);
}

int conv_wgrad_partials(const __nv_bfloat16* x, const __nv_bfloat16* dy, float* partial, const ConvShape& s, bool stem,
                        int* splits_out, cudaStream_t st) {
  if (int rc = check_shape(s, stem, "conv_wgrad")) return rc;
  IgemmParams P{};
  P.src = x; P.n = s.n; P.hs = s.h; P.ws = s.w; P.cs = s.cin; P.hm = s.ho; P.wm = s.wo;
  P.kh = s.kh; P.kw = s.kw; P.stride = s.stride; P.pad = s.pad; P.transposed = 0;
  P.cpb = stem ? 1 : s.cin / 64;
  P.pixels = static_cast<long long>(s.n) * s.ho * s.wo;
  P.num_kblocks = static_cast<int>((P.pixels + 63) / 64);
  P.total_chunks = s.kh * s.kw * s.cin / 64;
  P.ntaps_c = s.kh * s.kw;
  DIRB_CHECK_ARG(stem || P.ntaps_c <= kMaxTaps, "conv_wgrad: at most %d filter taps (got %dx%d)", kMaxTaps, s.kh, s.kw);
  for (int i = 0; i < kMaxTaps; ++i) P.tap_list[i] = i;
  const int splits = conv_wgrad_splits(s);
  P.kblocks_per_split = (P.num_kblocks + splits - 1) / splits;
  P.ldc = s.cout; P.out = partial;
  const int bn = wgrad_bn(s);
  P.n_tiles = s.cout / bn;
  const int m_tiles = (P.total_chunks + 1) / 2;
  *splits_out = splits;
  CUtensorMap tm;
  if (int rc = make_tmap_bf16_2d(&tm, dy, s.cout, static_cast<uint64_t>(P.pixels), static_cast<uint64_t>(s.cout) * 2, 64))
    return rc;
  if (stem) return DISPATCH_BN(bn, true, true, tm, P, m_tiles, splits, st);
  if (is_plain_gemm(s, stem)) {
    CUtensorMap ta;
    if (int rc = make_tmap_bf16_2d(&ta, x, s.cin, static_cast<uint64_t>(P.pixels), static_cast<uint64_t>(s.cin) * 2, 64))
      return rc;
    P.a_mode = 1;
    return DISPATCH_BN(bn, true, false, tm, P, m_tiles, splits, st, &ta);
  }
  if (im2col_enabled()) {
    CUtensorMap ta;
    if (int rc = make_tmap_im2col_bf16(&ta, x, s.cin, s.w, s.h, s.n, -s.pad, -s.pad, s.pad - (s.kw - 1),
                                       s.pad - (s.kh - 1), s.stride, 64))
      return rc;
    P.a_mode = 2; P.i2c_stride = s.stride; P.i2c_lo = -s.pad;
    return DISPATCH_BN(bn, true, false, tm, P, m_tiles, splits, st, &ta);
  }
  return DISPATCH_BN(bn, true, false, tm, P, m_tiles, splits, st);
}

int check_upsampled_conv(int n, int h, int w, int cin, int cout, int ho, int wo, const char* who) {
  DIRB_CHECK_ARG(n > 0 && h > 0 && w > 0 && ho > 0 && wo > 0, "%s: sizes must be positive", who);
  DIRB_CHECK_ARG(ho >= h && wo >= w, "%s: the target size must be at least the source size (%dx%d -> %dx%d)", who, h, w,
                 ho, wo);
  DIRB_CHECK_ARG(cin > 0 && cin % 64 == 0, "%s: Cin must be a positive multiple of 64 (got %d)", who, cin);
  DIRB_CHECK_ARG(cout > 0 && cout % 64 == 0, "%s: Cout must be a positive multiple of 64 (got %d)", who, cout);
  DIRB_CHECK_ARG(n <= 8192 && ho <= 512 && wo <= 512, "%s: at most 8192 images of at most 512 x 512 (got %d x %dx%d)",
                 who, n, ho, wo);
  DIRB_CHECK_ARG(static_cast<long long>(n) * ho * wo < (1LL << 31), "%s: more than 2^31 pixels", who);
  return DIRB200_OK;
}

static ConvShape upsampled_shape(int n, int cin, int cout, int ho, int wo) {
  return ConvShape{n, ho, wo, cin, cout, 5, 5, 1, 2, ho, wo};
}

static IgemmParams upsampled_params(const __nv_bfloat16* x, int n, int h, int w, int cin, int ho, int wo) {
  IgemmParams P{};
  P.src = x; P.n = n; P.hs = ho; P.ws = wo; P.cs = cin; P.hm = ho; P.wm = wo;
  P.kh = 5; P.kw = 5; P.stride = 1; P.pad = 2; P.transposed = 0;
  P.cpb = cin / 64;
  P.pixels = static_cast<long long>(n) * ho * wo;
  P.ntaps_c = 25;
  for (int i = 0; i < kMaxTaps; ++i) P.tap_list[i] = i;
  P.up_h = h; P.up_w = w;
  P.up_sh = static_cast<float>(h) / ho;
  P.up_sw = static_cast<float>(w) / wo;
  return P;
}

template <int BN, bool WGRAD>
static int launch_upsampled(const CUtensorMap& tm, const IgemmParams& P, int m_tiles, int splits, cudaStream_t st) {
  IgemmParams Q = P;
  Q.m_tiles = m_tiles;
  Q.num_tiles = m_tiles * P.n_tiles * splits;
  return launch_igemm_impl<BN, WGRAD, false, false, false, false, true>(tm, tm, Q, st);
}

int conv_fprop_upsampled(const __nv_bfloat16* x, const __nv_bfloat16* w_fprop, __nv_bfloat16* y, int n, int h, int w,
                         int cin, int cout, int ho, int wo, cudaStream_t st) {
  if (int rc = check_upsampled_conv(n, h, w, cin, cout, ho, wo, "conv_fprop_upsampled")) return rc;
  const ConvShape s = upsampled_shape(n, cin, cout, ho, wo);
  if (int rc = check_shape(s, false, "conv_fprop_upsampled")) return rc;
  const int ktot = 25 * cin;
  IgemmParams P = upsampled_params(x, n, h, w, cin, ho, wo);
  P.num_kblocks = ktot / 64;
  P.ldc = cout; P.out = y;
  const int m_tiles = static_cast<int>((P.pixels + BM - 1) / BM);
  const int bn = pick_bn(cout);
  P.n_tiles = cout / bn;
  CUtensorMap tm;
  if (int rc = make_tmap_bf16_2d(&tm, w_fprop, ktot, cout, static_cast<uint64_t>(ktot) * 2, bn)) return rc;
  return bn == 128 ? launch_upsampled<128, false>(tm, P, m_tiles, 1, st) : launch_upsampled<64, false>(tm, P, m_tiles, 1, st);
}

size_t conv_wgrad_upsampled_workspace_bytes(int n, int cin, int cout, int ho, int wo) {
  return conv_wgrad_workspace_bytes(upsampled_shape(n, cin, cout, ho, wo));
}

int conv_wgrad_partials_upsampled(const __nv_bfloat16* x, const __nv_bfloat16* dy, float* partial, int n, int h, int w,
                                  int cin, int cout, int ho, int wo, int* splits_out, cudaStream_t st) {
  if (int rc = check_upsampled_conv(n, h, w, cin, cout, ho, wo, "conv_wgrad_upsampled")) return rc;
  const ConvShape s = upsampled_shape(n, cin, cout, ho, wo);
  if (int rc = check_shape(s, false, "conv_wgrad_upsampled")) return rc;
  IgemmParams P = upsampled_params(x, n, h, w, cin, ho, wo);
  P.num_kblocks = static_cast<int>((P.pixels + 63) / 64);
  P.total_chunks = 25 * cin / 64;
  const int splits = conv_wgrad_splits(s);
  P.kblocks_per_split = (P.num_kblocks + splits - 1) / splits;
  P.ldc = cout; P.out = partial;
  const int bn = wgrad_bn(s);
  P.n_tiles = cout / bn;
  const int m_tiles = (P.total_chunks + 1) / 2;
  *splits_out = splits;
  CUtensorMap tm;
  if (int rc = make_tmap_bf16_2d(&tm, dy, cout, static_cast<uint64_t>(P.pixels), static_cast<uint64_t>(cout) * 2, 64))
    return rc;
  return bn == 128 ? launch_upsampled<128, true>(tm, P, m_tiles, splits, st)
                   : launch_upsampled<64, true>(tm, P, m_tiles, splits, st);
}

int conv_plan(const ConvShape& s, bool stem, int op, int* plan) {
  for (int i = 0; i < 7; ++i) plan[i] = 0;
  plan[4] = plan[5] = 1;
  if (int rc = check_shape(s, stem, "conv_plan")) return rc;
  if (op == 2) {
    plan[0] = wgrad_bn(s);
    plan[4] = conv_wgrad_splits(s);
    plan[2] = stem ? 0 : (is_plain_gemm(s, stem) ? 1 : (im2col_enabled() ? 2 : 0));
    return DIRB200_OK;
  }
  const bool dgrad = op == 1;
  DIRB_CHECK_ARG(!(dgrad && stem), "conv_plan: the stem has no data gradient");
  const int n_dim = dgrad ? s.cin : s.cout;
  plan[0] = pick_bn(n_dim);
  if (dgrad && s.stride == 2) {
    int launches = 0;
    for (int cls = 0; cls < 4; ++cls) {
      const int py = cls >> 1, px = cls & 1;
      int nt = 0;
      for (int r = 0; r < s.kh; ++r)
        for (int q = 0; q < s.kw; ++q)
          if (((py + s.pad - r) & 1) == 0 && ((px + s.pad - q) & 1) == 0) ++nt;
      const int hm = (s.h - py + 1) / 2, wm = (s.w - px + 1) / 2;
      if (nt == 0 || hm <= 0 || wm <= 0) continue;
      ++launches;
    }
    plan[2] = im2col_enabled() ? 2 : 0; plan[5] = launches;
    return DIRB200_OK;
  }
  const bool tma_fed = is_plain_gemm(s, stem) || (!stem && im2col_enabled() && (!dgrad || s.kh == s.kw));
  plan[2] = stem ? 0 : (is_plain_gemm(s, stem) ? 1 : (tma_fed ? 2 : 0));
  plan[6] = dgrad && conv_dgrad_fuses_bn_moments(s);
  return DIRB200_OK;
}

}
```

imbalanced-regression_b200/csrc/resnet_runner.cu:

```cuda
#include <stdlib.h>
#include <vector>
#include "common.cuh"
#include "conv.cuh"
#include "nn.cuh"

namespace dirb200 {

struct BNLayer {
  int c = 0;
  size_t gamma_off = 0, beta_off = 0;
  size_t rm_off = 0, rv_off = 0;
  float *mean = nullptr, *invstd = nullptr, *scale = nullptr, *shift = nullptr, *coef = nullptr;
};

struct ConvLayer {
  ConvShape s{};
  bool stem = false;
  size_t w_off = 0;
  __nv_bfloat16 *wf = nullptr, *wd = nullptr;
  float* wpart = nullptr;
  __nv_bfloat16* y = nullptr;
  __nv_bfloat16* a = nullptr;
  int64_t rows = 0;
  BNLayer bn;
};

struct Block {
  ConvLayer c1, c2, c3, ds;
  bool has_ds = false;
  const __nv_bfloat16* in = nullptr;
  __nv_bfloat16* out = nullptr;
  uint8_t* mask = nullptr;
};

}

using namespace dirb200;

struct dirb200_net {
  int n = 0, h = 0, w = 0;
  ConvLayer stem;
  std::vector<Block> blocks;
  __nv_bfloat16 *x_s2d = nullptr, *pool_out = nullptr;
  uint8_t* pool_idx = nullptr;
  int pool_h = 0, pool_w = 0;
  int feat_c = 0, feat_hw = 0;
  __nv_bfloat16* scratch[8] = {};
  WgradReduceDesc* reduce_descs = nullptr;
  std::vector<int> reduce_begin;
  float* bn_partial = nullptr;
  float* stat_partial = nullptr;
  PrepDesc* prep_descs = nullptr;
  BnEvalDesc* bn_eval_descs = nullptr;
  int num_bns = 0, max_bn_c = 0;
  int num_convs = 0;
  size_t param_count = 0, running_count = 0, activation_bytes = 0;
  std::vector<void*> allocs;
  bool forward_was_training = false;
  std::vector<int> stage_begin;
  int bwd_next_stage = -1;
  __nv_bfloat16 *bw_gA = nullptr, *bw_gB = nullptr, *bw_nA = nullptr, *bw_nB = nullptr, *bw_spareB = nullptr;
  int bw_gB_h = 0, bw_gB_w = 0;
  struct GraphSlot {
    cudaGraphExec_t exec = nullptr;
    const void *k0 = nullptr, *k1 = nullptr;
    int warm = 0;
    int64_t launches = 0;
    __nv_bfloat16 *gA = nullptr, *gB = nullptr, *nA = nullptr, *nB = nullptr, *spareB = nullptr;
    int gB_h = 0, gB_w = 0;
  };
  GraphSlot g_fwd, g_bwd[6];
  GraphSlot g_fwd_blocks, g_bwd_blocks[6][6][2];
  bool bwd_blocks = false;
  int bwd_top = -1;
  cudaStream_t cap_stream = nullptr;
  float *enc_buf = nullptr, *denc_buf = nullptr;
  bool profiling = false;
  struct ProfRec { int kind; cudaEvent_t a, b; };
  std::vector<ProfRec> prof;
  std::vector<cudaEvent_t> event_pool;
};

namespace dirb200 {

static bool dev_alloc(dirb200_net* net, void** p, size_t bytes) {
  if (cudaMalloc(p, bytes) != cudaSuccess) {
    set_error("resnet_create: cudaMalloc of %zu bytes failed", bytes);
    return false;
  }
  net->allocs.push_back(*p);
  net->activation_bytes += bytes;
  return true;
}

#define NET_ALLOC(ptr, bytes)                                                     \
  do {                                                                            \
    if (!dev_alloc(net, reinterpret_cast<void**>(&(ptr)), (bytes))) return false; \
  } while (0)

static bool setup_bn(dirb200_net* net, BNLayer& bn, int c) {
  bn.c = c;
  bn.gamma_off = net->param_count;
  bn.beta_off = net->param_count + c;
  net->param_count += 2 * (size_t)c;
  bn.rm_off = net->running_count;
  bn.rv_off = net->running_count + c;
  net->running_count += 2 * (size_t)c;
  float* f = nullptr;
  NET_ALLOC(f, sizeof(float) * 7 * c);
  bn.mean = f; bn.invstd = f + c; bn.scale = f + 2 * c; bn.shift = f + 3 * c; bn.coef = f + 4 * c;
  return true;
}

static bool setup_conv(dirb200_net* net, ConvLayer& cv, int n, int h, int w, int cin, int cout, int k, int stride,
                       int pad, bool stem, bool with_act) {
  cv.stem = stem;
  const int ho = (h + 2 * pad - k) / stride + 1, wo = (w + 2 * pad - k) / stride + 1;
  if (stem) cv.s = ConvShape{n, h / 2, w / 2, 16, cout, 4, 4, 1, 2, h / 2, w / 2};
  else cv.s = ConvShape{n, h, w, cin, cout, k, k, stride, pad, ho, wo};
  cv.w_off = net->param_count;
  net->param_count += (size_t)cout * cin * k * k;
  cv.rows = (int64_t)n * ho * wo;
  const size_t welems = stem ? (size_t)cout * 256 : (size_t)cout * cin * k * k;
  NET_ALLOC(cv.wf, welems * 2);
  if (!stem) NET_ALLOC(cv.wd, welems * 2);
  NET_ALLOC(cv.wpart, conv_wgrad_workspace_bytes(cv.s));
  NET_ALLOC(cv.y, (size_t)cv.rows * cout * 2);
  if (with_act) NET_ALLOC(cv.a, (size_t)cv.rows * cout * 2);
  return setup_bn(net, cv.bn, cout);
}

static bool build(dirb200_net* net, const int* blocks_per_stage, int num_stages) {
  const int n = net->n;
  if (!setup_conv(net, net->stem, n, net->h, net->w, 3, 64, 7, 2, 3, true, false)) return false;
  int h = net->h / 2, w = net->w / 2;
  NET_ALLOC(net->x_s2d, (size_t)n * h * w * 16 * 2);
  net->pool_h = (h - 1) / 2 + 1;
  net->pool_w = (w - 1) / 2 + 1;
  const size_t pool_elems = (size_t)n * net->pool_h * net->pool_w * 64;
  NET_ALLOC(net->pool_out, pool_elems * 2);
  NET_ALLOC(net->pool_idx, pool_elems);
  h = net->pool_h; w = net->pool_w;
  int inplanes = 64;
  const __nv_bfloat16* cur = net->pool_out;
  size_t max_act = (size_t)net->stem.rows * 64;
  net->stage_begin.assign(1, 0);
  for (int st = 0; st < num_stages; ++st) {
    const int planes = 64 << st;
    net->stage_begin.push_back((int)net->blocks.size());
    for (int b = 0; b < blocks_per_stage[st]; ++b) {
      const int stride = (b == 0 && st > 0) ? 2 : 1;
      net->blocks.emplace_back();
      Block& B = net->blocks.back();
      B.in = cur;
      B.has_ds = (b == 0) && (stride != 1 || inplanes != planes * 4);
      if (!setup_conv(net, B.c1, n, h, w, inplanes, planes, 1, 1, 0, false, true)) return false;
      if (!setup_conv(net, B.c2, n, h, w, planes, planes, 3, stride, 1, false, true)) return false;
      const int h2 = B.c2.s.ho, w2 = B.c2.s.wo;
      if (!setup_conv(net, B.c3, n, h2, w2, planes, planes * 4, 1, 1, 0, false, false)) return false;
      if (B.has_ds && !setup_conv(net, B.ds, n, h, w, inplanes, planes * 4, 1, stride, 0, false, false)) return false;
      NET_ALLOC(B.out, (size_t)B.c3.rows * planes * 4 * 2);
      NET_ALLOC(B.mask, (size_t)B.c3.rows * planes * 4 / 8);
      max_act = std::max(max_act, (size_t)B.c1.rows * std::max(inplanes, planes));
      max_act = std::max(max_act, (size_t)B.c3.rows * planes * 4);
      cur = B.out;
      inplanes = planes * 4;
      h = h2; w = w2;
    }
  }
  net->stage_begin.push_back((int)net->blocks.size());
  net->feat_c = inplanes;
  net->feat_hw = h * w;
  for (int i = 0; i < 8; ++i) NET_ALLOC(net->scratch[i], max_act * 2);
  {
    std::vector<WgradReduceDesc> rd;
    auto addr = [&](const ConvLayer& cv) {
      rd.push_back(WgradReduceDesc{cv.wpart, cv.w_off, conv_wgrad_splits(cv.s), cv.s.cout, cv.stem ? 3 : cv.s.cin,
                                   cv.stem ? 7 : cv.s.kh, cv.stem ? 7 : cv.s.kw, cv.stem ? 1 : 0});
    };
    net->reduce_begin.clear();
    net->reduce_begin.push_back(0);
    addr(net->stem);
    for (int stg = 1; stg <= num_stages; ++stg) {
      net->reduce_begin.push_back((int)rd.size());
      for (int bi = net->stage_begin[stg]; bi < net->stage_begin[stg + 1]; ++bi) {
        Block& B = net->blocks[bi];
        addr(B.c1); addr(B.c2); addr(B.c3);
        if (B.has_ds) addr(B.ds);
      }
    }
    net->reduce_begin.push_back((int)rd.size());
    NET_ALLOC(net->reduce_descs, sizeof(WgradReduceDesc) * rd.size());
    if (cudaMemcpy(net->reduce_descs, rd.data(), sizeof(WgradReduceDesc) * rd.size(), cudaMemcpyHostToDevice) != cudaSuccess)
      return false;
  }
  NET_ALLOC(net->enc_buf, sizeof(float) * (size_t)n * net->feat_c);
  NET_ALLOC(net->denc_buf, sizeof(float) * (size_t)n * net->feat_c);
  NET_ALLOC(net->bn_partial, sizeof(float) * bn_partial_floats(net->feat_c));
  NET_ALLOC(net->stat_partial, sizeof(float) * bn_partial_floats(net->feat_c));
  std::vector<PrepDesc> descs;
  auto add = [&](const ConvLayer& cv) {
    descs.push_back(make_prep_desc(cv.w_off, cv.s.cout, cv.stem ? 3 : cv.s.cin, cv.stem ? 7 : cv.s.kh, cv.stem ? 7 : cv.s.kw,
                                   cv.stem ? 1 : 0, cv.wf, cv.wd));
  };
  add(net->stem);
  for (Block& B : net->blocks) {
    add(B.c1); add(B.c2); add(B.c3);
    if (B.has_ds) add(B.ds);
  }
  net->num_convs = (int)descs.size();
  NET_ALLOC(net->prep_descs, sizeof(PrepDesc) * descs.size());
  if (cudaMemcpy(net->prep_descs, descs.data(), sizeof(PrepDesc) * descs.size(), cudaMemcpyHostToDevice) != cudaSuccess)
    return false;
  std::vector<BnEvalDesc> bd;
  auto addbn = [&](const BNLayer& bn) {
    bd.push_back(BnEvalDesc{bn.c, bn.gamma_off, bn.beta_off, bn.rm_off, bn.rv_off, bn.scale, bn.shift});
    net->max_bn_c = std::max(net->max_bn_c, bn.c);
  };
  addbn(net->stem.bn);
  for (Block& B : net->blocks) {
    addbn(B.c1.bn); addbn(B.c2.bn); addbn(B.c3.bn);
    if (B.has_ds) addbn(B.ds.bn);
  }
  net->num_bns = (int)bd.size();
  NET_ALLOC(net->bn_eval_descs, sizeof(BnEvalDesc) * bd.size());
  return cudaMemcpy(net->bn_eval_descs, bd.data(), sizeof(BnEvalDesc) * bd.size(), cudaMemcpyHostToDevice) == cudaSuccess;
}

#define RUN(expr)                    \
  do {                               \
    if (int _rc = (expr)) return _rc; \
  } while (0)

enum ProfKind { kPrep = 0, kFprop, kDgrad, kWgrad, kWgradReduce, kBnStats, kBnApply, kBnBwdReduce, kBnBwdApply, kPool,
                kNumProfKinds };

static cudaEvent_t prof_event(dirb200_net* net) {
  if (!net->event_pool.empty()) {
    cudaEvent_t e = net->event_pool.back();
    net->event_pool.pop_back();
    return e;
  }
  cudaEvent_t e;
  cudaEventCreate(&e);
  return e;
}
static inline void prof_begin(dirb200_net* net, int kind, cudaStream_t st) {
  if (!net->profiling) return;
  dirb200_net::ProfRec r{kind, prof_event(net), prof_event(net)};
  cudaEventRecord(r.a, st);
  net->prof.push_back(r);
}
static inline void prof_end(dirb200_net* net, cudaStream_t st) {
  if (!net->profiling) return;
  cudaEventRecord(net->prof.back().b, st);
}
#define RUNP(kind, expr)          \
  do {                            \
    prof_begin(net, (kind), st);  \
    int _rc = (expr);             \
    prof_end(net, st);            \
    if (_rc) return _rc;          \
  } while (0)

static bool fused_stats() {
  static const bool on = [] {
    const char* e = getenv("DIRB200_FUSED_STATS");
    return !(e != nullptr && e[0] == '0');
  }();
  return on;
}

static int conv_bn_forward(dirb200_net* net, ConvLayer& cv, const __nv_bfloat16* in, const float* params,
                           float* running, bool training, cudaStream_t st) {
  BNLayer& bn = cv.bn;
  if (training) {
    StatLayout lay{};
    const bool fused = fused_stats();
    RUNP(kFprop, conv_fprop(in, cv.wf, cv.y, cv.s, cv.stem, st, fused ? net->stat_partial : nullptr, &lay));
    if (!fused) {
      int nblk = 0;
      RUNP(kBnStats, bn_stats(cv.y, cv.rows, bn.c, net->stat_partial, &nblk, st));
      lay = StatLayout{nblk, 1, bn.c, 1};
    }
    RUNP(kBnStats, bn_finalize(net->stat_partial, lay, cv.rows, bn.c, params + bn.gamma_off, params + bn.beta_off, 1e-5f,
                               0.1f, running ? running + bn.rm_off : nullptr, running ? running + bn.rv_off : nullptr,
                               bn.mean, bn.invstd, bn.scale, bn.shift, st));
  } else {
    RUNP(kFprop, conv_fprop(in, cv.wf, cv.y, cv.s, cv.stem, st));
    RUNP(kBnStats, bn_eval_coeffs(bn.c, params + bn.gamma_off, params + bn.beta_off, 1e-5f, running + bn.rm_off,
                                  running + bn.rv_off, bn.scale, bn.shift, st));
  }
  if (cv.a)
    RUNP(kBnApply, bn_apply(cv.y, bn.scale, bn.shift, nullptr, nullptr, nullptr, nullptr, true, cv.rows, bn.c, cv.a, nullptr, st));
  return DIRB200_OK;
}

static int wgrad_step(dirb200_net* net, const __nv_bfloat16* x, const __nv_bfloat16* dy, ConvLayer& cv, cudaStream_t st) {
  int splits = 1;
  RUNP(kWgrad, conv_wgrad_partials(x, dy, cv.wpart, cv.s, cv.stem, &splits, st));
  return DIRB200_OK;
}

static int wgrad_reduce_stage(dirb200_net* net, int stage, float* grads, cudaStream_t st) {
  const int lo = net->reduce_begin[stage], hi = net->reduce_begin[stage + 1];
  RUNP(kWgradReduce, wgrad_reduce_all(net->reduce_descs + lo, hi - lo, grads, st));
  return DIRB200_OK;
}

static int conv_bn_backward(dirb200_net* net, ConvLayer& cv, const __nv_bfloat16* g, const float* params, float* grads,
                            __nv_bfloat16* dy, cudaStream_t st, const StatLayout* moments = nullptr) {
  BNLayer& bn = cv.bn;
  if (moments) {
    RUNP(kBnBwdApply, bn_bwd_coeffs_layout(net->bn_partial, *moments, cv.rows, bn.c, bn.mean, bn.invstd,
                                           params + bn.gamma_off, grads + bn.gamma_off, grads + bn.beta_off, bn.coef, st));
  } else {
    int nblk = 0;
    RUNP(kBnBwdReduce, bn_bwd_reduce(g, nullptr, cv.y, nullptr, bn.scale, bn.shift, nullptr, cv.rows, bn.c,
                                     net->bn_partial, &nblk, st));
    RUNP(kBnBwdApply, bn_bwd_coeffs(net->bn_partial, nblk, 2, 1, cv.rows, bn.c, bn.mean, bn.invstd,
                                    params + bn.gamma_off, grads + bn.gamma_off, grads + bn.beta_off, bn.coef, st));
  }
  RUNP(kBnBwdApply, bn_bwd_apply(g, nullptr, cv.y, bn.coef, nullptr, nullptr, bn.scale, bn.shift, nullptr, cv.rows, bn.c,
                                 dy, nullptr, nullptr, st));
  return DIRB200_OK;
}

static bool folded_eval() {
  static const bool on = [] {
    const char* e = getenv("DIRB200_FOLDED_EVAL");
    return !(e != nullptr && e[0] == '0');
  }();
  return on;
}

static int forward_eval_folded(dirb200_net* net, const float* params, const float* running, float* enc_out,
                               cudaStream_t st) {
  RUNP(kBnStats, bn_eval_coeffs_all(net->bn_eval_descs, net->num_bns, net->max_bn_c, params, running, 1e-5f, st));
  RUNP(kFprop, conv_fprop(net->x_s2d, net->stem.wf, net->stem.y, net->stem.s, true, st));
  RUNP(kPool, bn_relu_maxpool_fwd(net->stem.y, net->stem.bn.scale, net->stem.bn.shift, net->n, net->stem.s.ho,
                                  net->stem.s.wo, 64, net->pool_out, net->pool_idx, st));
  for (Block& B : net->blocks) {
    RUNP(kFprop, conv_fprop_affine(B.in, B.c1.wf, B.c1.a, B.c1.s, ConvEpilogue{B.c1.bn.scale, B.c1.bn.shift, nullptr, true}, st));
    RUNP(kFprop, conv_fprop_affine(B.c1.a, B.c2.wf, B.c2.a, B.c2.s, ConvEpilogue{B.c2.bn.scale, B.c2.bn.shift, nullptr, true}, st));
    const __nv_bfloat16* shortcut = B.in;
    if (B.has_ds) {
      RUNP(kFprop, conv_fprop_affine(B.in, B.ds.wf, B.ds.y, B.ds.s, ConvEpilogue{B.ds.bn.scale, B.ds.bn.shift, nullptr, false}, st));
      shortcut = B.ds.y;
    }
    RUNP(kFprop, conv_fprop_affine(B.c2.a, B.c3.wf, B.out, B.c3.s, ConvEpilogue{B.c3.bn.scale, B.c3.bn.shift, shortcut, true}, st));
  }
  if (enc_out) RUNP(kPool, avgpool_fwd(net->blocks.back().out, net->n, net->feat_hw, net->feat_c, enc_out, st));
  return DIRB200_OK;
}

static int forward_body(dirb200_net* net, const float* params, float* running, bool tr, float* enc_out,
                        cudaStream_t st) {
  RUN(conv_bn_forward(net, net->stem, net->x_s2d, params, running, tr, st));
  RUNP(kPool, bn_relu_maxpool_fwd(net->stem.y, net->stem.bn.scale, net->stem.bn.shift, net->n, net->stem.s.ho,
                                  net->stem.s.wo, 64, net->pool_out, net->pool_idx, st));
  for (Block& B : net->blocks) {
    RUN(conv_bn_forward(net, B.c1, B.in, params, running, tr, st));
    RUN(conv_bn_forward(net, B.c2, B.c1.a, params, running, tr, st));
    RUN(conv_bn_forward(net, B.c3, B.c2.a, params, running, tr, st));
    if (B.has_ds) {
      RUN(conv_bn_forward(net, B.ds, B.in, params, running, tr, st));
      RUNP(kBnApply, bn_apply(B.c3.y, B.c3.bn.scale, B.c3.bn.shift, nullptr, B.ds.y, B.ds.bn.scale, B.ds.bn.shift, true,
                              B.c3.rows, B.c3.bn.c, B.out, tr ? B.mask : nullptr, st));
    } else {
      RUNP(kBnApply, bn_apply(B.c3.y, B.c3.bn.scale, B.c3.bn.shift, B.in, nullptr, nullptr, nullptr, true, B.c3.rows,
                              B.c3.bn.c, B.out, tr ? B.mask : nullptr, st));
    }
  }
  if (enc_out) RUNP(kPool, avgpool_fwd(net->blocks.back().out, net->n, net->feat_hw, net->feat_c, enc_out, st));
  return DIRB200_OK;
}

static int check_blocks_mode(const dirb200_net* net, const char* who) {
  const int nst = (int)net->stage_begin.size() - 2;
  for (int s = 1; s <= nst; ++s)
    DIRB_CHECK_ARG(!net->blocks[net->stage_begin[s + 1] - 1].has_ds,
                   "%s: layer group %d ends in a downsample block; multi-scale mode needs an identity block there", who, s);
  return DIRB200_OK;
}

static bool graphs_enabled() {
  static const bool on = [] {
    const char* e = getenv("DIRB200_GRAPH");
    return !(e != nullptr && e[0] == '0');
  }();
  return on;
}

template <typename F>
static int run_graphed(dirb200_net* net, dirb200_net::GraphSlot& g, const void* k0, const void* k1, cudaStream_t st,
                       F&& body) {
  if (!graphs_enabled() || net->profiling) return body(st);
  if (g.exec && g.k0 == k0 && g.k1 == k1) {
    DIRB_CUDA(cudaGraphLaunch(g.exec, st));
    g_launches.fetch_add(g.launches);
    return DIRB200_OK;
  }
  if (g.exec) {
    cudaGraphExecDestroy(g.exec);
    g.exec = nullptr;
    g.warm = 0;
  }
  if (g.warm == 0 || g.k0 != k0 || g.k1 != k1) {
    g.k0 = k0; g.k1 = k1; g.warm = 1;
    return body(st);
  }
  const int64_t before = g_launches.load();
  if (!net->cap_stream) DIRB_CUDA(cudaStreamCreateWithFlags(&net->cap_stream, cudaStreamNonBlocking));
  DIRB_CUDA(cudaStreamBeginCapture(net->cap_stream, cudaStreamCaptureModeThreadLocal));
  const int rc = body(net->cap_stream);
  cudaGraph_t graph = nullptr;
  const cudaError_t e = cudaStreamEndCapture(net->cap_stream, &graph);
  if (rc != DIRB200_OK || e != cudaSuccess || graph == nullptr) {
    if (graph) cudaGraphDestroy(graph);
    if (rc == DIRB200_OK) set_error("resnet: stream capture failed (%s)", cudaGetErrorString(e));
    (void)cudaGetLastError();
    return rc != DIRB200_OK ? rc : DIRB200_ERR_CUDA;
  }
  g.launches = g_launches.load() - before;
  g_launches.fetch_sub(g.launches);
  const cudaError_t ei = cudaGraphInstantiate(&g.exec, graph, 0);
  cudaGraphDestroy(graph);
  if (ei != cudaSuccess) {
    g.exec = nullptr;
    set_error("resnet: cudaGraphInstantiate failed (%s)", cudaGetErrorString(ei));
    return DIRB200_ERR_CUDA;
  }
  DIRB_CUDA(cudaGraphLaunch(g.exec, st));
  g_launches.fetch_add(g.launches);
  return DIRB200_OK;
}

static bool fused_bwd_moments() {
  static const bool on = [] {
    const char* e = getenv("DIRB200_FUSED_BWD_MOMENTS");
    return !(e != nullptr && e[0] == '0');
  }();
  return on;
}

static int dgrad_with_bn_moments(dirb200_net* net, const __nv_bfloat16* dy, ConvLayer& cv, ConvLayer& prev,
                                 __nv_bfloat16* g, StatLayout* lay, bool* fused, cudaStream_t st) {
  *fused = fused_bwd_moments() && conv_dgrad_fuses_bn_moments(cv.s);
  if (!*fused) {
    RUNP(kDgrad, conv_dgrad(dy, cv.wd, g, cv.s, st));
    return DIRB200_OK;
  }
  const DgradBnMoments bm{prev.y, prev.bn.scale, prev.bn.shift, net->bn_partial, lay};
  RUNP(kDgrad, conv_dgrad(dy, cv.wd, g, cv.s, st, &bm));
  return DIRB200_OK;
}

}

static constexpr int kMaxNetBatch = 1 << 13;
static constexpr int kMaxNetSide = 2 * (1 << 9);

extern "C" {

int dirb200_resnet_create(int n, int h, int w, const int* blocks_per_stage, int num_stages, dirb200_net** out) {
  DIRB_CHECK_ARG(out && blocks_per_stage && n > 0 && num_stages >= 1 && num_stages <= 4, "resnet_create: bad arguments");
  DIRB_CHECK_ARG(h > 0 && w > 0 && h % 4 == 0 && w % 4 == 0, "resnet_create: H and W must be multiples of 4 (got %dx%d)",
                 h, w);
  DIRB_CHECK_ARG(n <= kMaxNetBatch, "resnet_create: N must be at most %d (got %d)", kMaxNetBatch, n);
  DIRB_CHECK_ARG(h <= kMaxNetSide && w <= kMaxNetSide, "resnet_create: H and W must be at most %d (got %dx%d)", kMaxNetSide,
                 h, w);
  DIRB_CHECK_ARG((int64_t)n * (h / 2) * (w / 2) < (int64_t(1) << 31),
                 "resnet_create: N * H/2 * W/2 must be below 2^31 (got %d x %d x %d)", n, h / 2, w / 2);
  dirb200_net* net = new dirb200_net();
  net->n = n; net->h = h; net->w = w;
  if (!build(net, blocks_per_stage, num_stages)) {
    for (void* p : net->allocs) cudaFree(p);
    delete net;
    return DIRB200_ERR_CUDA;
  }
  *out = net;
  return DIRB200_OK;
}

void dirb200_resnet_destroy(dirb200_net* net) {
  if (!net) return;
  if (net->cap_stream) cudaStreamDestroy(net->cap_stream);
  if (net->g_fwd.exec) cudaGraphExecDestroy(net->g_fwd.exec);
  if (net->g_fwd_blocks.exec) cudaGraphExecDestroy(net->g_fwd_blocks.exec);
  for (auto& g : net->g_bwd)
    if (g.exec) cudaGraphExecDestroy(g.exec);
  for (auto& per_stage : net->g_bwd_blocks)
    for (auto& per_top : per_stage)
      for (auto& g : per_top)
        if (g.exec) cudaGraphExecDestroy(g.exec);
  for (void* p : net->allocs) cudaFree(p);
  delete net;
}

int64_t dirb200_resnet_param_count(const dirb200_net* net) { return net ? (int64_t)net->param_count : -1; }
int64_t dirb200_resnet_running_count(const dirb200_net* net) { return net ? (int64_t)net->running_count : -1; }
int64_t dirb200_resnet_feature_dim(const dirb200_net* net) { return net ? net->feat_c : -1; }
int64_t dirb200_resnet_device_bytes(const dirb200_net* net) { return net ? (int64_t)net->activation_bytes : -1; }

int dirb200_resnet_set_profiling(dirb200_net* net, int enabled) {
  DIRB_CHECK_ARG(net, "resnet_set_profiling: null net");
  net->profiling = enabled != 0;
  return DIRB200_OK;
}

int dirb200_resnet_read_profile(dirb200_net* net, double* ms_by_kind, int64_t* groups_by_kind) {
  DIRB_CHECK_ARG(net && ms_by_kind && groups_by_kind, "resnet_read_profile: null pointer");
  for (int i = 0; i < kNumProfKinds; ++i) { ms_by_kind[i] = 0.0; groups_by_kind[i] = 0; }
  for (auto& r : net->prof) {
    DIRB_CUDA(cudaEventSynchronize(r.b));
    float ms = 0.f;
    DIRB_CUDA(cudaEventElapsedTime(&ms, r.a, r.b));
    ms_by_kind[r.kind] += ms;
    groups_by_kind[r.kind] += 1;
    net->event_pool.push_back(r.a);
    net->event_pool.push_back(r.b);
  }
  net->prof.clear();
  return DIRB200_OK;
}

int dirb200_resnet_forward(dirb200_net* net, const float* x_nchw, const float* params, float* bn_running, int training,
                           float* enc_out, void* stream) {
  DIRB_CHECK_ARG(net && x_nchw && params && enc_out, "resnet_forward: null pointer");
  DIRB_CHECK_ARG(training || bn_running, "resnet_forward: eval mode needs the running statistics");
  cudaStream_t st = as_stream(stream);
  const bool tr = training != 0;
  RUNP(kPrep, prep_weights_all(params, net->prep_descs, net->num_convs, st));
  RUNP(kPrep, input_to_s2d(x_nchw, net->n, net->h, net->w, net->x_s2d, st));
  if (!tr && folded_eval()) {
    RUN(forward_eval_folded(net, params, bn_running, enc_out, st));
    net->forward_was_training = false;
    return DIRB200_OK;
  }
  const bool graphed = tr && graphs_enabled() && !net->profiling;
  float* enc_dst = graphed ? net->enc_buf : enc_out;
  auto body = [&](cudaStream_t st) -> int { return forward_body(net, params, bn_running, tr, enc_dst, st); };
  if (graphed) {
    RUN(run_graphed(net, net->g_fwd, params, bn_running, st, body));
    DIRB_CUDA(cudaMemcpyAsync(enc_out, net->enc_buf, sizeof(float) * (size_t)net->n * net->feat_c,
                              cudaMemcpyDeviceToDevice, st));
  } else {
    RUN(body(st));
  }
  net->forward_was_training = tr;
  return DIRB200_OK;
}

int dirb200_resnet_forward_blocks(dirb200_net* net, const float* x_nchw, const float* params, float* bn_running,
                                  int training, void* const* block_out, void* stream) {
  DIRB_CHECK_ARG(net && x_nchw && params && block_out, "resnet_forward_blocks: null pointer");
  DIRB_CHECK_ARG(training || bn_running, "resnet_forward_blocks: eval mode needs the running statistics");
  const int nst = (int)net->stage_begin.size() - 2;
  for (int s = 0; s < nst; ++s) DIRB_CHECK_ARG(block_out[s], "resnet_forward_blocks: null block_out[%d]", s);
  RUN(check_blocks_mode(net, "resnet_forward_blocks"));
  cudaStream_t st = as_stream(stream);
  const bool tr = training != 0;
  RUNP(kPrep, prep_weights_all(params, net->prep_descs, net->num_convs, st));
  RUNP(kPrep, input_to_s2d(x_nchw, net->n, net->h, net->w, net->x_s2d, st));
  if (!tr && folded_eval()) {
    RUN(forward_eval_folded(net, params, bn_running, nullptr, st));
  } else {
    auto body = [&](cudaStream_t st) -> int { return forward_body(net, params, bn_running, tr, nullptr, st); };
    if (tr) RUN(run_graphed(net, net->g_fwd_blocks, params, bn_running, st, body));
    else RUN(body(st));
  }
  for (int s = 0; s < nst; ++s) {
    const Block& B = net->blocks[net->stage_begin[s + 2] - 1];
    DIRB_CUDA(cudaMemcpyAsync(block_out[s], B.out, sizeof(__nv_bfloat16) * (size_t)B.c3.rows * B.c3.s.cout,
                              cudaMemcpyDeviceToDevice, st));
  }
  net->forward_was_training = tr;
  return DIRB200_OK;
}

}

namespace dirb200 {

static int backward_blocks(dirb200_net* net, int lo, int hi, const float* params, float* grads, cudaStream_t st,
                           const __nv_bfloat16* g3 = nullptr) {
  __nv_bfloat16 *gA = net->bw_gA, *gB = net->bw_gB, *nA = net->bw_nA, *nB = net->bw_nB, *spareB = net->bw_spareB;
  __nv_bfloat16 *t1 = net->scratch[4], *t2 = net->scratch[5], *t3 = net->scratch[6];
  int gB_h = net->bw_gB_h, gB_w = net->bw_gB_w;
  for (int bi = hi - 1; bi >= lo; --bi) {
    Block& B = net->blocks[bi];
    BNLayer& b3 = B.c3.bn;
    int nblk = 0;
    const int kparts = B.has_ds ? 3 : 2;
    RUNP(kBnBwdReduce, bn_bwd_reduce(gA, gB, B.c3.y, B.has_ds ? B.ds.y : nullptr, nullptr, nullptr, B.mask, B.c3.rows,
                                     b3.c, net->bn_partial, &nblk, st, gB_h, gB_w, B.has_ds ? nullptr : nB,
                                     bi == hi - 1 ? g3 : nullptr));
    if (B.has_ds) {
      BNLayer& bd = B.ds.bn;
      RUNP(kBnBwdApply, bn_bwd_coeffs(net->bn_partial, nblk, kparts, 2, B.c3.rows, b3.c, bd.mean, bd.invstd,
                                      params + bd.gamma_off, grads + bd.gamma_off, grads + bd.beta_off, bd.coef, st));
    }
    RUNP(kBnBwdApply, bn_bwd_coeffs(net->bn_partial, nblk, kparts, 1, B.c3.rows, b3.c, b3.mean, b3.invstd,
                                    params + b3.gamma_off, grads + b3.gamma_off, grads + b3.beta_off, b3.coef, st));
    if (B.has_ds)
      RUNP(kBnBwdApply, bn_bwd_apply(gA, gB, B.c3.y, b3.coef, B.ds.y, B.ds.bn.coef, nullptr, nullptr, B.mask, B.c3.rows,
                                     b3.c, t1, t2, nullptr, st, gB_h, gB_w));
    else
      RUNP(kBnBwdApply, bn_bwd_apply(nB, nullptr, B.c3.y, b3.coef, nullptr, nullptr, nullptr, nullptr, nullptr, B.c3.rows,
                                     b3.c, t1, nullptr, nullptr, st));
    gB_h = gB_w = 0;
    RUN(wgrad_step(net, B.c2.a, t1, B.c3, st));
    StatLayout mlay{};
    bool mfused = false;
    RUN(dgrad_with_bn_moments(net, t1, B.c3, B.c2, t3, &mlay, &mfused, st));
    RUN(conv_bn_backward(net, B.c2, t3, params, grads, t1, st, mfused ? &mlay : nullptr));
    RUN(wgrad_step(net, B.c1.a, t1, B.c2, st));
    RUN(dgrad_with_bn_moments(net, t1, B.c2, B.c1, t3, &mlay, &mfused, st));
    RUN(conv_bn_backward(net, B.c1, t3, params, grads, t1, st, mfused ? &mlay : nullptr));
    RUN(wgrad_step(net, B.in, t1, B.c1, st));
    RUNP(kDgrad, conv_dgrad(t1, B.c1.wd, nA, B.c1.s, st));
    if (B.has_ds) {
      RUN(wgrad_step(net, B.in, t2, B.ds, st));
      const ConvShape& d = B.ds.s;
      if (d.stride == 2 && d.kh == 1 && d.kw == 1 && d.pad == 0 && d.h % 2 == 0 && d.w % 2 == 0 && bi > 0 &&
          !net->blocks[bi - 1].has_ds) {
        const ConvShape cs{d.n, d.ho, d.wo, d.cin, d.cout, 1, 1, 1, 0, d.ho, d.wo};
        RUNP(kDgrad, conv_dgrad(t2, B.ds.wd, nB, cs, st));
        gB_h = d.h;
        gB_w = d.w;
      } else {
        RUNP(kDgrad, conv_dgrad(t2, B.ds.wd, nB, B.ds.s, st));
      }
    }
    __nv_bfloat16* oldA = gA;
    __nv_bfloat16* oldB = gB ? gB : spareB;
    gA = nA; gB = nB;
    nA = oldA; nB = oldB;
    spareB = nullptr;
  }
  net->bw_gA = gA; net->bw_gB = gB; net->bw_nA = nA; net->bw_nB = nB; net->bw_spareB = spareB;
  net->bw_gB_h = gB_h; net->bw_gB_w = gB_w;
  return DIRB200_OK;
}

static int backward_stage_run(dirb200_net* net, int stage, const float* params, float* grads, const __nv_bfloat16* g3,
                              dirb200_net::GraphSlot& g, cudaStream_t st) {
  auto body = [&](cudaStream_t st) -> int {
    if (stage >= 1) {
      RUN(backward_blocks(net, net->stage_begin[stage], net->stage_begin[stage + 1], params, grads, st, g3));
    } else {
      __nv_bfloat16 *t1 = net->scratch[4], *t3 = net->scratch[6];
      RUNP(kPool, maxpool_bwd(net->bw_gA, net->bw_gB, net->pool_idx, net->n, net->stem.s.ho, net->stem.s.wo, 64, t3, st));
      RUN(conv_bn_backward(net, net->stem, t3, params, grads, t1, st));
      RUN(wgrad_step(net, net->x_s2d, t1, net->stem, st));
    }
    RUN(wgrad_reduce_stage(net, stage, grads, st));
    return DIRB200_OK;
  };
  if (!graphs_enabled() || net->profiling) return body(st);
  const bool replay = g.exec && g.k0 == params && g.k1 == grads;
  RUN(run_graphed(net, g, params, grads, st, body));
  if (replay) {
    net->bw_gA = g.gA; net->bw_gB = g.gB; net->bw_nA = g.nA; net->bw_nB = g.nB; net->bw_spareB = g.spareB;
    net->bw_gB_h = g.gB_h; net->bw_gB_w = g.gB_w;
  } else {
    g.gA = net->bw_gA; g.gB = net->bw_gB; g.nA = net->bw_nA; g.nB = net->bw_nB; g.spareB = net->bw_spareB;
    g.gB_h = net->bw_gB_h; g.gB_w = net->bw_gB_w;
  }
  return DIRB200_OK;
}

}

extern "C" {

int dirb200_resnet_backward_stage(dirb200_net* net, int stage, const float* d_enc, const float* params, float* grads,
                                  void* stream) {
  DIRB_CHECK_ARG(net && params && grads, "resnet_backward_stage: null pointer");
  const int nst = (int)net->stage_begin.size() - 2;
  DIRB_CHECK_ARG(stage >= 0 && stage <= nst, "resnet_backward_stage: bad stage %d", stage);
  cudaStream_t st = as_stream(stream);
  if (stage == nst) {
    DIRB_CHECK_ARG(net->forward_was_training, "resnet_backward: needs a preceding training-mode forward");
    DIRB_CHECK_ARG(d_enc, "resnet_backward_stage: the first stage needs d_enc");
    net->bw_gA = net->scratch[0]; net->bw_gB = nullptr; net->bw_nA = net->scratch[2]; net->bw_nB = net->scratch[3];
    net->bw_spareB = net->scratch[1];
    net->bw_gB_h = net->bw_gB_w = 0;
    RUNP(kPool, avgpool_bwd(d_enc, net->n, net->feat_hw, net->feat_c, net->bw_gA, st));
  } else {
    DIRB_CHECK_ARG(net->bwd_next_stage == stage && !net->bwd_blocks,
                   "resnet_backward_stage: stage %d out of order (expected %d%s)", stage, net->bwd_next_stage,
                   net->bwd_blocks ? " of a multi-scale backward" : "");
  }
  net->bwd_next_stage = -1;
  net->bwd_blocks = false;
  RUN(backward_stage_run(net, stage, params, grads, nullptr, net->g_bwd[stage], st));
  net->bwd_next_stage = stage - 1;
  return DIRB200_OK;
}

int dirb200_resnet_backward_blocks_stage(dirb200_net* net, int stage, const void* d_block, const float* params,
                                         float* grads, void* stream) {
  DIRB_CHECK_ARG(net && params && grads, "resnet_backward_blocks_stage: null pointer");
  const int nst = (int)net->stage_begin.size() - 2;
  DIRB_CHECK_ARG(stage >= 0 && stage <= nst, "resnet_backward_blocks_stage: bad stage %d", stage);
  DIRB_CHECK_ARG(stage > 0 || !d_block, "resnet_backward_blocks_stage: stage 0 (the stem) takes no block gradient");
  RUN(check_blocks_mode(net, "resnet_backward_blocks_stage"));
  cudaStream_t st = as_stream(stream);
  if (stage == nst) {
    DIRB_CHECK_ARG(net->forward_was_training, "resnet_backward_blocks_stage: needs a preceding training-mode forward");
    net->bwd_top = -1;
  } else {
    DIRB_CHECK_ARG(net->bwd_next_stage == stage && net->bwd_blocks,
                   "resnet_backward_blocks_stage: stage %d out of order (expected %d%s)", stage, net->bwd_next_stage,
                   net->bwd_blocks ? "" : " of a multi-scale backward");
  }
  net->bwd_next_stage = -1;
  net->bwd_blocks = true;
  const __nv_bfloat16* g3 = nullptr;
  if (stage > 0 && d_block) {
    const Block& B = net->blocks[net->stage_begin[stage + 1] - 1];
    const size_t bytes = sizeof(__nv_bfloat16) * (size_t)B.c3.rows * B.c3.s.cout;
    if (net->bwd_top < 0) {
      net->bwd_top = stage;
      net->bw_gA = net->scratch[0]; net->bw_gB = nullptr; net->bw_nA = net->scratch[2]; net->bw_nB = net->scratch[3];
      net->bw_spareB = net->scratch[1];
      net->bw_gB_h = net->bw_gB_w = 0;
      DIRB_CUDA(cudaMemcpyAsync(net->bw_gA, d_block, bytes, cudaMemcpyDeviceToDevice, st));
    } else {
      DIRB_CUDA(cudaMemcpyAsync(net->scratch[7], d_block, bytes, cudaMemcpyDeviceToDevice, st));
      g3 = net->scratch[7];
    }
  }
  if (net->bwd_top >= 0)
    RUN(backward_stage_run(net, stage, params, grads, g3, net->g_bwd_blocks[stage][net->bwd_top][g3 ? 1 : 0], st));
  net->bwd_next_stage = stage - 1;
  if (stage == 0) net->bwd_blocks = false;
  return DIRB200_OK;
}

int dirb200_resnet_stage_param_range(const dirb200_net* net, int stage, int64_t* lo, int64_t* hi) {
  DIRB_CHECK_ARG(net && lo && hi, "resnet_stage_param_range: null pointer");
  const int nst = (int)net->stage_begin.size() - 2;
  DIRB_CHECK_ARG(stage >= 0 && stage <= nst, "resnet_stage_param_range: bad stage %d", stage);
  auto first = [&](int s) -> int64_t {
    return s > nst ? (int64_t)net->param_count : (int64_t)net->blocks[net->stage_begin[s]].c1.w_off;
  };
  *lo = stage == 0 ? 0 : first(stage);
  *hi = first(stage + 1);
  return DIRB200_OK;
}

int dirb200_resnet_num_stages(const dirb200_net* net) { return net ? (int)net->stage_begin.size() - 2 : -1; }

int dirb200_resnet_backward(dirb200_net* net, const float* d_enc, const float* params, float* grads, void* stream) {
  DIRB_CHECK_ARG(net && d_enc && params && grads, "resnet_backward: null pointer");
  for (int stage = (int)net->stage_begin.size() - 2; stage >= 0; --stage)
    RUN(dirb200_resnet_backward_stage(net, stage, d_enc, params, grads, stream));
  return DIRB200_OK;
}

}

extern "C" {
int dirb200_resnet_peek(dirb200_net* net, int block, int which, void** ptr, int64_t* rows, int* channels) {
  DIRB_CHECK_ARG(net && ptr && rows && channels, "resnet_peek: null pointer");
  DIRB_CHECK_ARG(block >= -1 && block < (int)net->blocks.size(), "resnet_peek: bad block %d", block);
  const ConvLayer* cv = nullptr;
  bool act = false;
  if (block < 0) {
    if (which == 6) {
      *ptr = net->pool_out; *rows = (int64_t)net->n * net->pool_h * net->pool_w; *channels = 64;
      return DIRB200_OK;
    }
    cv = &net->stem; act = which == 1;
  } else {
    Block& B = net->blocks[block];
    switch (which) {
      case 0: cv = &B.c1; break;
      case 1: cv = &B.c1; act = true; break;
      case 2: cv = &B.c2; break;
      case 3: cv = &B.c2; act = true; break;
      case 4: cv = &B.c3; break;
      case 5: DIRB_CHECK_ARG(B.has_ds, "resnet_peek: block has no downsample"); cv = &B.ds; break;
      case 6: *ptr = B.out; *rows = B.c3.rows; *channels = B.c3.s.cout; return DIRB200_OK;
      default: DIRB_CHECK_ARG(false, "resnet_peek: bad selector %d", which);
    }
  }
  *ptr = act ? cv->a : cv->y;
  *rows = cv->rows;
  *channels = cv->s.cout;
  DIRB_CHECK_ARG(*ptr, "resnet_peek: tensor not materialised");
  return DIRB200_OK;
}
}
```

imbalanced-regression_b200/csrc/tc.cuh:

```cuda
#pragma once
#include <cuda.h>
#include <stdint.h>

namespace dirb200 {
namespace tc {

__device__ __forceinline__ uint32_t smem_u32(const void* p) {
  return static_cast<uint32_t>(__cvta_generic_to_shared(p));
}

__device__ __forceinline__ void mbar_init(uint32_t bar, uint32_t count) {
  asm volatile("mbarrier.init.shared::cta.b64 [%0], %1;" ::"r"(bar), "r"(count) : "memory");
}
__device__ __forceinline__ void fence_barrier_init() {
  asm volatile("fence.mbarrier_init.release.cluster;" ::: "memory");
}
__device__ __forceinline__ void mbar_arrive(uint32_t bar) {
  asm volatile("mbarrier.arrive.shared::cta.b64 _, [%0];" ::"r"(bar) : "memory");
}
__device__ __forceinline__ void mbar_arrive_expect_tx(uint32_t bar, uint32_t bytes) {
  asm volatile("mbarrier.arrive.expect_tx.shared::cta.b64 _, [%0], %1;" ::"r"(bar), "r"(bytes) : "memory");
}
__device__ __forceinline__ bool mbar_try_wait(uint32_t bar, uint32_t parity) {
  uint32_t ok;
  asm volatile(
      "{\n"
      ".reg .pred p;\n"
      "mbarrier.try_wait.parity.shared::cta.b64 p, [%1], %2;\n"
      "selp.u32 %0, 1, 0, p;\n"
      "}\n"
      : "=r"(ok)
      : "r"(bar), "r"(parity)
      : "memory");
  return ok != 0;
}
__device__ __forceinline__ void mbar_wait(uint32_t bar, uint32_t parity) {
  if (mbar_try_wait(bar, parity)) return;
  unsigned long long t0;
  asm volatile("mov.u64 %0, %%globaltimer;" : "=l"(t0));
  while (!mbar_try_wait(bar, parity)) {
    unsigned long long t1;
    asm volatile("mov.u64 %0, %%globaltimer;" : "=l"(t1));
    if (t1 - t0 > 4000000000ull) __trap();
  }
}

__device__ __forceinline__ bool elect_one() {
  uint32_t pred;
  asm volatile(
      "{\n"
      ".reg .pred P;\n"
      "elect.sync _|P, 0xffffffff;\n"
      "selp.u32 %0, 1, 0, P;\n"
      "}\n"
      : "=r"(pred));
  return pred != 0;
}

__device__ __forceinline__ void cp_async16(uint32_t dst, const void* src, uint32_t src_bytes) {
  asm volatile("cp.async.cg.shared.global [%0], [%1], 16, %2;" ::"r"(dst), "l"(src), "r"(src_bytes) : "memory");
}
__device__ __forceinline__ void cp_async_mbar_arrive_noinc(uint32_t bar) {
  asm volatile("cp.async.mbarrier.arrive.noinc.shared::cta.b64 [%0];" ::"r"(bar) : "memory");
}
__device__ __forceinline__ void fence_proxy_async() { asm volatile("fence.proxy.async.shared::cta;" ::: "memory"); }

__device__ __forceinline__ void tma_load_2d(uint32_t dst, const CUtensorMap* tmap, uint32_t bar, int c0, int c1) {
  asm volatile(
      "cp.async.bulk.tensor.2d.shared::cluster.global.mbarrier::complete_tx::bytes [%0], [%1, {%3, %4}], [%2];"
      ::"r"(dst), "l"(tmap), "r"(bar), "r"(c0), "r"(c1)
      : "memory");
}

__device__ __forceinline__ void tma_load_im2col_4d(uint32_t dst, const CUtensorMap* tmap, uint32_t bar, int c, int w,
                                                   int h, int n, uint16_t off_w, uint16_t off_h) {
  asm volatile(
      "cp.async.bulk.tensor.4d.shared::cluster.global.im2col.mbarrier::complete_tx::bytes"
      " [%0], [%1, {%3, %4, %5, %6}], [%2], {%7, %8};"
      ::"r"(dst), "l"(tmap), "r"(bar), "r"(c), "r"(w), "r"(h), "r"(n), "h"(off_w), "h"(off_h)
      : "memory");
}

__device__ __forceinline__ void wgmma_fence() { asm volatile("wgmma.fence.sync.aligned;" ::: "memory"); }
__device__ __forceinline__ void wgmma_commit() { asm volatile("wgmma.commit_group.sync.aligned;" ::: "memory"); }
template <int N>
__device__ __forceinline__ void wgmma_wait() {
  asm volatile("wgmma.wait_group.sync.aligned %0;" ::"n"(N) : "memory");
}
template <int R>
__device__ __forceinline__ void wgmma_fence_operands(float (&d)[R]) {
#pragma unroll
  for (int i = 0; i < R; ++i) asm volatile("" : "+f"(d[i])::"memory");
}

#define DIRB_F4(i) "+f"(d[i]), "+f"(d[i + 1]), "+f"(d[i + 2]), "+f"(d[i + 3])
#define DIRB_F16(i) DIRB_F4(i), DIRB_F4(i + 4), DIRB_F4(i + 8), DIRB_F4(i + 12)
#define DIRB_R8(a, b, c, e, f, g, h, k) "%" #a ", %" #b ", %" #c ", %" #e ", %" #f ", %" #g ", %" #h ", %" #k ", "
template <int TA, int TB>
__device__ __forceinline__ void wgmma_m64n64(float (&d)[32], uint64_t adesc, uint64_t bdesc, uint32_t accumulate) {
  asm volatile(
      "{\n.reg .pred p;\nsetp.ne.b32 p, %34, 0;\n"
      "wgmma.mma_async.sync.aligned.m64n64k16.f32.bf16.bf16 {"
      DIRB_R8(0, 1, 2, 3, 4, 5, 6, 7) DIRB_R8(8, 9, 10, 11, 12, 13, 14, 15) DIRB_R8(16, 17, 18, 19, 20, 21, 22, 23)
      "%24, %25, %26, %27, %28, %29, %30, %31}, %32, %33, p, 1, 1, %35, %36;\n}\n"
      : DIRB_F16(0), DIRB_F16(16)
      : "l"(adesc), "l"(bdesc), "r"(accumulate), "n"(TA), "n"(TB));
}
template <int TA, int TB>
__device__ __forceinline__ void wgmma_m64n128(float (&d)[64], uint64_t adesc, uint64_t bdesc, uint32_t accumulate) {
  asm volatile(
      "{\n.reg .pred p;\nsetp.ne.b32 p, %66, 0;\n"
      "wgmma.mma_async.sync.aligned.m64n128k16.f32.bf16.bf16 {"
      DIRB_R8(0, 1, 2, 3, 4, 5, 6, 7) DIRB_R8(8, 9, 10, 11, 12, 13, 14, 15) DIRB_R8(16, 17, 18, 19, 20, 21, 22, 23)
      DIRB_R8(24, 25, 26, 27, 28, 29, 30, 31) DIRB_R8(32, 33, 34, 35, 36, 37, 38, 39) DIRB_R8(40, 41, 42, 43, 44, 45, 46, 47)
      DIRB_R8(48, 49, 50, 51, 52, 53, 54, 55)
      "%56, %57, %58, %59, %60, %61, %62, %63}, %64, %65, p, 1, 1, %67, %68;\n}\n"
      : DIRB_F16(0), DIRB_F16(16), DIRB_F16(32), DIRB_F16(48)
      : "l"(adesc), "l"(bdesc), "r"(accumulate), "n"(TA), "n"(TB));
}
#undef DIRB_R8
#undef DIRB_F16
#undef DIRB_F4
template <int BN, int TA, int TB>
__device__ __forceinline__ void wgmma_bf16(float (&d)[BN / 2], uint64_t adesc, uint64_t bdesc, uint32_t accumulate) {
  if constexpr (BN == 128) wgmma_m64n128<TA, TB>(d, adesc, bdesc, accumulate);
  else wgmma_m64n64<TA, TB>(d, adesc, bdesc, accumulate);
}

__device__ __forceinline__ uint64_t make_smem_desc(uint32_t saddr, uint32_t lbo_bytes, uint32_t sbo_bytes) {
  uint64_t d = 0;
  d |= static_cast<uint64_t>((saddr & 0x3FFFFu) >> 4);
  d |= static_cast<uint64_t>((lbo_bytes >> 4) & 0x3FFFu) << 16;
  d |= static_cast<uint64_t>((sbo_bytes >> 4) & 0x3FFFu) << 32;
  d |= static_cast<uint64_t>(1) << 62;
  return d;
}

}
}
```

include/dirb200.h:

```cpp
#ifndef DIRB200_H
#define DIRB200_H

#include <stddef.h>
#include <stdint.h>

#ifdef __cplusplus
extern "C" {
#endif

#define DIRB200_OK 0
#define DIRB200_ERR_ARG (-1)
#define DIRB200_ERR_CUDA (-2)
#define DIRB200_ERR_WORKSPACE (-3)

#define DIRB200_BIN_AGE 0
#define DIRB200_BIN_DEPTH10 1
#define DIRB200_BIN_EDGES5 2

#define DIRB200_LOSS_MSE 0
#define DIRB200_LOSS_L1 1
#define DIRB200_LOSS_FOCAL_MSE 2
#define DIRB200_LOSS_FOCAL_L1 3
#define DIRB200_LOSS_HUBER 4
#define DIRB200_ACT_SIGMOID 0
#define DIRB200_ACT_TANH 1

#define DIRB200_REWEIGHT_SQRT_INV 1
#define DIRB200_REWEIGHT_INVERSE 2

const char* dirb200_last_error(void);
int dirb200_version(void);
int64_t dirb200_launch_count(void);


int dirb200_fds_label_flags(const float* labels, int64_t n, int bucket_num, int bucket_start,
                            int bin_rule, int32_t* flags, void* stream);

int dirb200_fds_bin_rows(const float* labels, int64_t n, int bucket_num, int bucket_start,
                         int bin_rule, const int32_t* flags, int32_t* bins_out, void* stream);

size_t dirb200_fds_accumulate_workspace_bytes(int64_t n, int nb);

int dirb200_fds_accumulate(const float* features, const int32_t* bins, int64_t n, int d, int nb,
                           double* sums, double* sumsq, int64_t* counts,
                           void* workspace, size_t workspace_bytes, void* stream);

int dirb200_fds_set_profiling(int enabled);
int dirb200_fds_last_accumulate_kernel_ms(float* ms_out);

int dirb200_fds_finalize(const double* sums, const double* sumsq, const int64_t* counts, int nb, int d,
                         float* running_mean, float* running_var, float* num_samples_tracked,
                         double momentum, int first_update, void* stream);

int dirb200_fds_smooth_tables(const float* src, int nb, int d, const float* window_host, int ks,
                              float* dst, void* stream);

int dirb200_fds_calibrate_fwd(float* x, const float* labels, int64_t b, int d, int bucket_num,
                              int bucket_start, int bin_rule, const float* m1, const float* v1,
                              const float* m2, const float* v2, float clip_min, float clip_max,
                              int32_t* rowbin_out, int32_t* flags_scratch ,
                              void* stream);

int dirb200_fds_fill_empty(const int64_t* counts, int nb, int d, float* running_mean, float* running_var,
                           void* stream);

int dirb200_fds_calibrate_bwd(int bin_rule, const float* grad_out, const int32_t* rowbin, int64_t b, int d,
                              const float* v1, const float* v2, float clip_min, float clip_max,
                              float* grad_in, void* stream);


size_t dirb200_loss_workspace_bytes(int64_t n);

int dirb200_loss_fwd_bwd(int kind, const float* pred, const float* target, const float* weight, int64_t n,
                         float beta, float gamma, int activate, float grad_scale,
                         float* loss_out, float* grad_out, void* workspace, size_t workspace_bytes,
                         void* stream);


int dirb200_lds_histogram(const float* labels, int64_t n, int max_target, int64_t* hist, void* stream);

int dirb200_lds_weights(const float* labels, int64_t n, int max_target, int reweight,
                        const double* window_host, int ks, const int64_t* hist,
                        double* scratch, float* weights_out, void* stream);

int dirb200_lds_weights_sharded(const float* labels, int64_t n, int64_t n_total, int max_target, int reweight,
                                const double* window_host, int ks, const int64_t* hist, double* scratch,
                                float* weights_out, void* stream);

int dirb200_lds_table_lookup(const float* values, int64_t n, float mult, int max_bin, const float* table,
                             float* weights_out, void* stream);

size_t dirb200_bn_workspace_bytes(int c);
int dirb200_bn_train_fwd(const void* y, int64_t rows, int c, const float* gamma, const float* beta, float eps,
                         float momentum, float* running_mean, float* running_var, int relu, void* out, float* save_mean,
                         float* save_invstd, float* scale_shift, void* workspace, void* stream);
int dirb200_bn_eval_coeffs(int c, const float* gamma, const float* beta, float eps, const float* running_mean,
                           const float* running_var, float* scale, float* shift, void* stream);
int dirb200_bn_train_bwd(const void* grad_out, const void* y, int64_t rows, int c, const float* gamma,
                         const float* save_mean, const float* save_invstd, const float* scale_shift, int relu,
                         float* grad_gamma, float* grad_beta, void* grad_y, void* workspace, void* stream);
int dirb200_maxpool3x3s2_fwd(const void* x, int n, int h, int w, int c, void* out, uint8_t* argmax, void* stream);
int dirb200_maxpool3x3s2_bwd(const void* grad_out, const uint8_t* argmax, int n, int h, int w, int c, void* grad_x,
                             void* stream);
int dirb200_avgpool_fwd(const void* x, int n, int hw, int c, float* out, void* stream);
int dirb200_avgpool_bwd(const float* grad_out, int n, int hw, int c, void* grad_x, void* stream);

int dirb200_upsample_bilinear_fwd(const void* x, int n, int h, int w, int c, int ho, int wo, void* out, void* stream);
int dirb200_upsample_bilinear_bwd(const void* dy, int n, int h, int w, int c, int ho, int wo, void* dx, void* stream);
int dirb200_copy_channels(const void* src, int src_stride, int src_off, void* dst, int dst_stride, int dst_off, int c,
                          int64_t pixels, void* stream);

int dirb200_augment_batch(const uint8_t* images, const int* crop_yx, const uint8_t* flip, int n, int size, int pad,
                          float mean, float stdv, float* out, void* stream);

int dirb200_int_label_histogram(const float* labels, int64_t n, int nbins, int64_t* hist, void* stream);

int dirb200_shot_metrics(const float* preds, const float* labels, int64_t n, const int64_t* train_hist, int nbins,
                         int many_shot_thr, int low_shot_thr, double* out16, void* stream);

size_t dirb200_depth_metrics_workspace_bytes(int64_t n_images, int h, int w);
int dirb200_depth_metrics_accumulate(const float* pred, int ph, int pw, const float* target, const uint8_t* mask,
                                     int64_t n_images, int h, int w, const uint8_t* group_of_bin, int nbins,
                                     double* acc, void* workspace, size_t workspace_bytes, void* stream);


int dirb200_conv_prep_weights(const float* w, int cout, int cin, int kh, int kw, int stem,
                              void* w_fprop, void* w_dgrad, void* stream);

int dirb200_input_to_s2d(const float* x_nchw, int n, int h, int w, void* out_bf16, void* stream);

int dirb200_conv_fprop(const void* x, const void* w_fprop, void* y, int n, int h, int w, int cin,
                       int cout, int kh, int kw, int stride, int pad, int stem, void* stream);

int dirb200_conv_dgrad(const void* dy, const void* w_dgrad, void* dx, int n, int h, int w, int cin,
                       int cout, int kh, int kw, int stride, int pad, void* stream);

int dirb200_conv_plan(int n, int h, int w, int cin, int cout, int kh, int kw, int stride, int pad, int stem, int op,
                      int* plan7);
size_t dirb200_conv_wgrad_workspace_bytes(int n, int h, int w, int cin, int cout, int kh, int kw,
                                          int stride, int pad, int stem);

int dirb200_conv_wgrad(const void* x, const void* dy, float* dw, void* workspace, size_t workspace_bytes,
                       int n, int h, int w, int cin, int cout, int kh, int kw, int stride, int pad,
                       int stem, int accumulate, void* stream);

int dirb200_conv_fprop_upsampled(const void* x, const void* w_fprop, void* y, int n, int h, int w, int cin, int cout,
                                 int ho, int wo, void* stream);
size_t dirb200_conv_wgrad_upsampled_workspace_bytes(int n, int h, int w, int cin, int cout, int ho, int wo);
int dirb200_conv_wgrad_upsampled(const void* x, const void* dy, float* dw, void* workspace, size_t workspace_bytes, int n,
                                 int h, int w, int cin, int cout, int ho, int wo, int accumulate, void* stream);


int dirb200_conv_fprop_bn_stats(const void* x, const void* w_fprop, void* y, int n, int h, int w, int cin, int cout,
                                int kh, int kw, int stride, int pad, int stem, float* partial, int* layout_host,
                                void* stream);
int dirb200_conv_fprop_affine(const void* x, const void* w_fprop, void* out, int n, int h, int w, int cin, int cout,
                              int kh, int kw, int stride, int pad, const float* scale, const float* shift,
                              const void* residual, int relu, void* stream);
int dirb200_conv_dgrad_bn_moments(const void* dy, const void* w_dgrad, void* dx, int n, int h, int w, int cin, int cout,
                                  int kh, int kw, int stride, int pad, const void* y_prev, const float* scale,
                                  const float* shift, float* partial, int* layout_host, void* stream);
int dirb200_bn_finalize_layout(const float* partial, const int* layout_host, int64_t rows, int c, const float* gamma,
                               const float* beta, float eps, float momentum, float* running_mean, float* running_var,
                               float* mean_out, float* invstd_out, float* scale_out, float* shift_out, void* stream);
int dirb200_bn_bwd_coeffs_layout(const float* partial, const int* layout_host, int64_t rows, int c, const float* mean,
                                 const float* invstd, const float* gamma, float* grad_gamma, float* grad_beta,
                                 float* coef_out, void* stream);


int dirb200_layer_bn_stats(const void* y, int64_t rows, int c, float* partial, int* nblocks_host, void* stream);
int dirb200_layer_bn_apply(const void* y, const float* scale, const float* shift, const void* res, const void* res_y,
                           const float* res_scale, const float* res_shift, int relu, int64_t rows, int c, void* out,
                           uint8_t* mask_out, void* stream);
int dirb200_layer_bn_bwd_reduce(const void* g1, const void* g2, const void* g3, const void* y, const void* y2,
                                const float* scale, const float* shift, const uint8_t* mask, int64_t rows, int c,
                                int g2_h, int g2_w, void* dz_out, float* partial, int* nblocks_host, void* stream);
int dirb200_layer_bn_bwd_coeffs(const float* partial, int nblocks, int k, int gslot, int64_t rows, int c,
                                const float* mean, const float* invstd, const float* gamma, float* grad_gamma,
                                float* grad_beta, float* coef_out, void* stream);
int dirb200_layer_bn_bwd_apply(const void* g1, const void* g2, const void* y, const float* coef, const void* y2,
                               const float* coef2, const float* scale, const float* shift, const uint8_t* mask,
                               int64_t rows, int c, int g2_h, int g2_w, void* dy, void* dy2, void* dz_out,
                               void* stream);
int dirb200_layer_bn_relu_maxpool_fwd(const void* y, const float* scale, const float* shift, int n, int h, int w, int c,
                                      void* out, uint8_t* argmax, void* stream);
int dirb200_layer_maxpool_bwd(const void* g1, const void* g2, const uint8_t* argmax, int n, int h, int w, int c,
                              void* dx, void* stream);

typedef struct dirb200_net dirb200_net;

int dirb200_resnet_create(int n, int h, int w, const int* blocks_per_stage, int num_stages, dirb200_net** out);
void dirb200_resnet_destroy(dirb200_net* net);
int64_t dirb200_resnet_param_count(const dirb200_net* net);
int64_t dirb200_resnet_running_count(const dirb200_net* net);
int64_t dirb200_resnet_feature_dim(const dirb200_net* net);
int64_t dirb200_resnet_device_bytes(const dirb200_net* net);

int dirb200_resnet_forward(dirb200_net* net, const float* x_nchw, const float* params, float* bn_running,
                           int training, float* enc_out, void* stream);

int dirb200_resnet_backward(dirb200_net* net, const float* d_enc, const float* params, float* grads, void* stream);

int dirb200_resnet_num_stages(const dirb200_net* net);
int dirb200_resnet_backward_stage(dirb200_net* net, int stage, const float* d_enc, const float* params, float* grads,
                                  void* stream);
int dirb200_resnet_stage_param_range(const dirb200_net* net, int stage, int64_t* lo, int64_t* hi);

int dirb200_resnet_forward_blocks(dirb200_net* net, const float* x_nchw, const float* params, float* bn_running,
                                  int training, void* const* block_out, void* stream);

int dirb200_resnet_backward_blocks_stage(dirb200_net* net, int stage, const void* d_block, const float* params,
                                         float* grads, void* stream);

int dirb200_resnet_set_profiling(dirb200_net* net, int enabled);
int dirb200_resnet_read_profile(dirb200_net* net, double* ms_by_kind, int64_t* groups_by_kind);

int dirb200_resnet_peek(dirb200_net* net, int block, int which, void** ptr, int64_t* rows, int* channels);

int dirb200_linear1_fwd(const float* x, const float* w, const float* bias, int64_t n, int d, float* pred,
                        void* stream);
int dirb200_linear1_bwd(const float* grad_pred, const float* x, const float* w, int64_t n, int d, float* dx,
                        float* dw, float* dbias, void* stream);

int dirb200_adam_step(float* params, const float* grads, float* exp_avg, float* exp_avg_sq, int64_t n, float lr,
                      float beta1, float beta2, float eps, float weight_decay, int64_t step, float grad_scale,
                      const float* clip_coef, void* stream);
int dirb200_sgd_step(float* params, const float* grads, float* momentum_buf, int64_t n, float lr, float momentum,
                     float weight_decay, int first_step, float grad_scale, const float* clip_coef, void* stream);

size_t dirb200_grad_clip_workspace_bytes(void);
int dirb200_grad_clip_coef(const float* grads, int64_t n, float grad_scale, float max_norm, void* workspace,
                           size_t workspace_bytes, float* out, void* stream);

#ifdef __cplusplus
}
#endif
#endif
```

Measured before the change: 7681.

## Apply BN+ReLU on operand load in fprop and wgrad GEMMs

Adds an APPLY variant of the implicit-GEMM kernel. It loads the raw pre-BN activation through ldmatrix into registers, applies the per-channel scale/shift and ReLU there, masks out padded taps, and feeds the result to register-sourced wgmma. In training the bottleneck blocks then pass raw conv outputs to the next conv's fprop and wgrad, so the separate bn_apply pass and its materialised activation are skipped. The cost is extra ALU work and register pressure in the main loop, RS-wgmma in place of SS, and a lazy bn_apply in the peek path.

```diff
diff --git a/imbalanced-regression_b200/_convlib.py b/imbalanced-regression_b200/_convlib.py
--- a/imbalanced-regression_b200/_convlib.py
+++ b/imbalanced-regression_b200/_convlib.py
@@ -22,4 +22,6 @@
     "dirb200_conv_dgrad_bn_moments": (c_int, [P, P, P] + _I9 + [P, P, P, P, P, P]),
     "dirb200_bn_finalize_layout": (c_int, [P, P, c_int64, c_int, P, P, c_float, c_float, P, P, P, P, P, P, P]),
     "dirb200_bn_bwd_coeffs_layout": (c_int, [P, P, c_int64, c_int, P, P, P, P, P, P, P]),
+    "dirb200_conv_fprop_apply": (c_int, [P] * 5 + _I9 + [P, P, P]),
+    "dirb200_conv_wgrad_apply": (c_int, [P] * 6 + [c_size_t] + _I9 + [c_int, P]),
 })
diff --git a/imbalanced-regression_b200/csrc/conv.cuh b/imbalanced-regression_b200/csrc/conv.cuh
--- a/imbalanced-regression_b200/csrc/conv.cuh
+++ b/imbalanced-regression_b200/csrc/conv.cuh
@@ -11,8 +11,14 @@
   int rows, n_tiles, bn, group;
 };
 
+struct ConvInputBn {
+  const float* scale;
+  const float* shift;
+};
+bool conv_applies_input_bn(const ConvShape& s);
 int conv_fprop(const __nv_bfloat16* x, const __nv_bfloat16* w, __nv_bfloat16* y, const ConvShape& s, bool stem,
-               cudaStream_t st, float* stat_partial = nullptr, StatLayout* layout = nullptr);
+               cudaStream_t st, float* stat_partial = nullptr, StatLayout* layout = nullptr,
+               const ConvInputBn* in_bn = nullptr);
 struct ConvEpilogue {
   const float* scale;
   const float* shift;
@@ -33,7 +39,7 @@
 int conv_wgrad_splits(const ConvShape& s);
 size_t conv_wgrad_workspace_bytes(const ConvShape& s);
 int conv_wgrad_partials(const __nv_bfloat16* x, const __nv_bfloat16* dy, float* partial, const ConvShape& s, bool stem,
-                        int* splits_out, cudaStream_t st);
+                        int* splits_out, cudaStream_t st, const ConvInputBn* in_bn = nullptr);
 int wgrad_reduce(const float* workspace, int splits, float* dw, const ConvShape& s, bool stem, bool accumulate,
                  cudaStream_t st);
 int check_upsampled_conv(int n, int h, int w, int cin, int cout, int ho, int wo, const char* who);
diff --git a/imbalanced-regression_b200/csrc/conv_api.cu b/imbalanced-regression_b200/csrc/conv_api.cu
--- a/imbalanced-regression_b200/csrc/conv_api.cu
+++ b/imbalanced-regression_b200/csrc/conv_api.cu
@@ -360,6 +360,40 @@
   return DIRB200_OK;
 }
 
+int dirb200_conv_fprop_apply(const void* y_prev, const float* scale, const float* shift, const void* w_fprop, void* y,
+                             int n, int h, int w, int cin, int cout, int kh, int kw, int stride, int pad, float* partial,
+                             int* layout_host, void* stream) {
+  DIRB_CHECK_ARG(y_prev && scale && shift && w_fprop && y && (!partial || layout_host), "conv_fprop_apply: null pointer");
+  ConvShape s;
+  if (int rc = to_shape(n, h, w, cin, cout, kh, kw, stride, pad, 0, &s)) return rc;
+  StatLayout lay{};
+  const ConvInputBn ib{scale, shift};
+  if (int rc = conv_fprop((const __nv_bfloat16*)y_prev, (const __nv_bfloat16*)w_fprop, (__nv_bfloat16*)y, s, false,
+                          as_stream(stream), partial, &lay, &ib))
+    return rc;
+  if (partial) layout_to_host(lay, layout_host);
+  return DIRB200_OK;
+}
+
+int dirb200_conv_wgrad_apply(const void* y_prev, const float* scale, const float* shift, const void* dy, float* dw,
+                             void* workspace, size_t workspace_bytes, int n, int h, int w, int cin, int cout, int kh,
+                             int kw, int stride, int pad, int accumulate, void* stream) {
+  DIRB_CHECK_ARG(y_prev && scale && shift && dy && dw && workspace, "conv_wgrad_apply: null pointer");
+  ConvShape s;
+  if (int rc = to_shape(n, h, w, cin, cout, kh, kw, stride, pad, 0, &s)) return rc;
+  if (workspace_bytes < conv_wgrad_workspace_bytes(s)) {
+    set_error("conv_wgrad_apply: workspace too small (%zu < %zu)", workspace_bytes, conv_wgrad_workspace_bytes(s));
+    return DIRB200_ERR_WORKSPACE;
+  }
+  cudaStream_t st = as_stream(stream);
+  int splits = 1;
+  const ConvInputBn ib{scale, shift};
+  if (int rc = conv_wgrad_partials((const __nv_bfloat16*)y_prev, (const __nv_bfloat16*)dy, (float*)workspace, s, false,
+                                   &splits, st, &ib))
+    return rc;
+  return wgrad_reduce((const float*)workspace, splits, dw, s, false, accumulate != 0, st);
+}
+
 int dirb200_conv_plan(int n, int h, int w, int cin, int cout, int kh, int kw, int stride, int pad, int stem, int op,
                       int* plan7) {
   DIRB_CHECK_ARG(plan7 && op >= 0 && op <= 2, "conv_plan: bad arguments");
diff --git a/imbalanced-regression_b200/csrc/conv_igemm.cu b/imbalanced-regression_b200/csrc/conv_igemm.cu
--- a/imbalanced-regression_b200/csrc/conv_igemm.cu
+++ b/imbalanced-regression_b200/csrc/conv_igemm.cu
@@ -47,6 +47,8 @@
   const float* bst_shift;
   int up_h, up_w;
   float up_sh, up_sw;
+  const float* in_scale;
+  const float* in_shift;
 };
 
 template <int BN, bool STAGED_EPI>
@@ -150,7 +152,27 @@
   }
   return out;
 }
-template <int BN, bool WGRAD, bool STEM, bool ATMA = false, bool AFFINE = false, bool BSTAT = false, bool UPS = false>
+
+__device__ __forceinline__ uint32_t fprop_tap_mask(const IgemmParams& P, long long p) {
+  if (p >= P.pixels) return 0u;
+  uint32_t n, rem, y, x;
+  P.fd_hw.divmod(static_cast<uint32_t>(p), n, rem);
+  P.fd_wm.divmod(rem, y, x);
+  const int yb = static_cast<int>(y) * P.stride - P.pad, xb = static_cast<int>(x) * P.stride - P.pad;
+  uint32_t vx = 0, m = 0;
+  for (int c = 0; c < P.kw; ++c) vx |= (static_cast<unsigned>(xb + c) < static_cast<unsigned>(P.ws) ? 1u : 0u) << c;
+  for (int r = 0; r < P.kh; ++r)
+    if (static_cast<unsigned>(yb + r) < static_cast<unsigned>(P.hs)) m |= vx << (r * P.kw);
+  return m;
+}
+__device__ __forceinline__ uint32_t bn_relu_bf2(uint32_t w, float sc0, float sc1, float sh0, float sh1, uint32_t keep) {
+  const float a = fmaxf(fmaf(__uint_as_float(w << 16), sc0, sh0), 0.f);
+  const float b = fmaxf(fmaf(__uint_as_float(w & 0xffff0000u), sc1, sh1), 0.f);
+  __nv_bfloat162 h = __floats2bfloat162_rn(a, b);
+  return *reinterpret_cast<uint32_t*>(&h) & keep;
+}
+template <int BN, bool WGRAD, bool STEM, bool ATMA = false, bool AFFINE = false, bool BSTAT = false, bool UPS = false,
+          bool APPLY = false>
 __global__ void __launch_bounds__(kThreads, 1)
 igemm_kernel(const __grid_constant__ CUtensorMap tmap_b, const __grid_constant__ CUtensorMap tmap_a,
              const IgemmParams P) {
@@ -160,6 +182,7 @@
   static_assert(!AFFINE || (!WGRAD && !STEM), "folded-BN epilogue: non-stem fprop GEMMs only");
   static_assert(!BSTAT || (ATMA && !WGRAD && !AFFINE), "BN-backward moments in the epilogue: TMA-fed dgrad GEMMs only");
   static_assert(!UPS || (!ATMA && !STEM && !AFFINE && !BSTAT), "up-sampled A operand: plain fprop / wgrad GEMMs only");
+  static_assert(!APPLY || (ATMA && !AFFINE && !BSTAT && !UPS), "BN + ReLU applied on load: TMA-fed fprop / wgrad only");
   extern __shared__ uint8_t smem_raw[];
   const uint32_t smem_base = (smem_u32(smem_raw) + 1023u) & ~1023u;
   uint8_t* const smem_gen = smem_raw + (smem_base - smem_u32(smem_raw));
@@ -519,6 +542,96 @@
     int split, m_tile, n_tile, kb_begin, nk;
     decode_tile(t, split, m_tile, n_tile, kb_begin, nk);
     int prev = 0;
+    if constexpr (APPLY) {
+      uint32_t tmask0 = 0, tmask1 = 0;
+      float wsc0 = 0.f, wsc1 = 0.f, wsh0 = 0.f, wsh1 = 0.f;
+      int chunk_r = 0, chunk_s = 0;
+      uint32_t lane_off;
+      if constexpr (!WGRAD) {
+        const long long p = static_cast<long long>(m_tile) * BM + g * 64 + wq * 16 + fr;
+        tmask0 = fprop_tap_mask(P, p);
+        tmask1 = fprop_tap_mask(P, p + 8);
+        lane_off = (wq * 16 + (lane & 15)) * 128;
+      } else {
+        const int gchunk = m_tile * 2 + g;
+        if (gchunk < P.total_chunks) {
+          uint32_t tap, cbk, cr, csx;
+          P.fd_cpb.divmod(static_cast<uint32_t>(gchunk), tap, cbk);
+          P.fd_kw.divmod(tap, cr, csx);
+          chunk_r = static_cast<int>(cr);
+          chunk_s = static_cast<int>(csx);
+          const int c = static_cast<int>(cbk) * 64 + wq * 16 + fr;
+          wsc0 = __ldg(P.in_scale + c); wsc1 = __ldg(P.in_scale + c + 8);
+          wsh0 = __ldg(P.in_shift + c); wsh1 = __ldg(P.in_shift + c + 8);
+        }
+        lane_off = ((lane >> 4) * 8 + (lane & 7)) * 128 + (((2 * wq + ((lane >> 3) & 1)) ^ (lane & 7)) << 4);
+      }
+      int tc = 0, cb = 0;
+      auto kblock = [&](int it, uint32_t (&a)[16]) {
+        const int s = static_cast<int>(rs);
+        mbar_wait(full_bar(s), rph);
+        if (++rs == nstages) { rs = 0; rph ^= 1u; }
+        const uint32_t base = a_addr(s) + g * 8192 + lane_off;
+#pragma unroll
+        for (int k = 0; k < BK / 16; ++k) {
+          if constexpr (!WGRAD) ldmatrix_x4(a + 4 * k, base + (((2 * k + (lane >> 4)) ^ (lane & 7)) << 4));
+          else ldmatrix_x4_trans(a + 4 * k, base + k * 2048);
+        }
+        if constexpr (!WGRAD) {
+          const int tap = P.tap_list[tc];
+          const uint32_t keep0 = ((tmask0 >> tap) & 1u) ? 0xffffffffu : 0u;
+          const uint32_t keep1 = ((tmask1 >> tap) & 1u) ? 0xffffffffu : 0u;
+          const int c0 = cb * 64 + fc;
+          if (++cb == P.cpb) { cb = 0; ++tc; }
+#pragma unroll
+          for (int j = 0; j < 8; ++j) {
+            const int c = c0 + 8 * j;
+            const float2 sc = __ldg(reinterpret_cast<const float2*>(P.in_scale + c));
+            const float2 sh = __ldg(reinterpret_cast<const float2*>(P.in_shift + c));
+            a[2 * j] = bn_relu_bf2(a[2 * j], sc.x, sc.y, sh.x, sh.y, keep0);
+            a[2 * j + 1] = bn_relu_bf2(a[2 * j + 1], sc.x, sc.y, sh.x, sh.y, keep1);
+          }
+        } else {
+          auto pixel_ok = [&](long long p) {
+            if (p >= P.pixels) return false;
+            uint32_t n, rem, y, x;
+            P.fd_hw.divmod(static_cast<uint32_t>(p), n, rem);
+            P.fd_wm.divmod(rem, y, x);
+            const int hi = static_cast<int>(y) * P.stride - P.pad + chunk_r, wi = static_cast<int>(x) * P.stride - P.pad + chunk_s;
+            return static_cast<unsigned>(hi) < static_cast<unsigned>(P.hs) && static_cast<unsigned>(wi) < static_cast<unsigned>(P.ws);
+          };
+          const long long p0 = static_cast<long long>(kb_begin + it) * 64 + lane;
+          const uint32_t vlo = __ballot_sync(0xffffffffu, pixel_ok(p0));
+          const uint32_t vhi = __ballot_sync(0xffffffffu, pixel_ok(p0 + 32));
+#pragma unroll
+          for (int j = 0; j < 8; ++j) {
+            const int kk = 8 * j + fc;
+            const uint32_t bits = (kk < 32 ? vlo >> kk : vhi >> (kk - 32)) & 3u;
+            const uint32_t keep = ((bits & 1u) ? 0x0000ffffu : 0u) | ((bits & 2u) ? 0xffff0000u : 0u);
+            a[2 * j] = bn_relu_bf2(a[2 * j], wsc0, wsc0, wsh0, wsh0, keep);
+            a[2 * j + 1] = bn_relu_bf2(a[2 * j + 1], wsc1, wsc1, wsh1, wsh1, keep);
+          }
+        }
+        const uint64_t bdesc = make_smem_desc(b_addr(s), kLbo, 1024u);
+        wgmma_fence_operands(acc);
+        wgmma_fence();
+#pragma unroll
+        for (int k = 0; k < BK / 16; ++k)
+          wgmma_bf16_rs<BN, kT>(acc, a + 4 * k, bdesc + static_cast<uint64_t>(k * kadv), (it > 0 || k > 0) ? 1u : 0u);
+        wgmma_commit();
+        wgmma_fence_operands(acc);
+        if (it > 0) {
+          wgmma_wait<1>();
+          if (lane == 0) mbar_arrive(empty_bar(prev));
+        }
+        prev = s;
+      };
+      uint32_t fa0[16], fa1[16];
+      for (int it = 0; it < nk; it += 2) {
+        kblock(it, fa0);
+        if (it + 1 < nk) kblock(it + 1, fa1);
+      }
+    } else
     for (int it = 0; it < nk; ++it) {
       const int s = static_cast<int>(rs);
       mbar_wait(full_bar(s), rph);
@@ -780,20 +893,21 @@
   return Q;
 }
 
-template <int BN, bool WGRAD, bool STEM, bool ATMA = false, bool AFFINE = false, bool BSTAT = false, bool UPS = false>
+template <int BN, bool WGRAD, bool STEM, bool ATMA = false, bool AFFINE = false, bool BSTAT = false, bool UPS = false,
+          bool APPLY = false>
 static int launch_igemm_impl(const CUtensorMap& tm, const CUtensorMap& tma, const IgemmParams& Qin, cudaStream_t st) {
   using C = Cfg<BN, !WGRAD>;
   const IgemmParams Q = finish_params(Qin);
   static bool configured = false;
   if (!configured) {
-    DIRB_CUDA(cudaFuncSetAttribute(igemm_kernel<BN, WGRAD, STEM, ATMA, AFFINE, BSTAT, UPS>,
+    DIRB_CUDA(cudaFuncSetAttribute(igemm_kernel<BN, WGRAD, STEM, ATMA, AFFINE, BSTAT, UPS, APPLY>,
                                    cudaFuncAttributeMaxDynamicSharedMemorySize, C::kSmemBytes));
     configured = true;
   }
   int grid = Q.num_tiles < num_sms() ? Q.num_tiles : num_sms();
   if (!WGRAD && grid < Q.n_tiles) grid = Q.n_tiles;
   t_last_layout = StatLayout{grid, Q.n_tiles, BN, 1};
-  igemm_kernel<BN, WGRAD, STEM, ATMA, AFFINE, BSTAT, UPS><<<grid, kThreads, C::kSmemBytes, st>>>(tm, tma, Q);
+  igemm_kernel<BN, WGRAD, STEM, ATMA, AFFINE, BSTAT, UPS, APPLY><<<grid, kThreads, C::kSmemBytes, st>>>(tm, tma, Q);
   DIRB_LAUNCHED();
   return DIRB200_OK;
 }
@@ -806,6 +920,8 @@
   Q.num_tiles = m_tiles * P.n_tiles * splits;
   if constexpr (!STEM) {
     if (tma) {
+      if (Q.in_scale != nullptr)
+        return launch_igemm_impl<BN, WGRAD, false, true, false, false, false, true>(tm, *tma, Q, st);
       if constexpr (!WGRAD) {
         if (Q.epi_scale != nullptr) return launch_igemm_impl<BN, false, false, true, true>(tm, *tma, Q, st);
         if (Q.bst_y != nullptr) return launch_igemm_impl<BN, false, false, true, false, true>(tm, *tma, Q, st);
@@ -816,8 +932,9 @@
   if constexpr (!WGRAD && !STEM) {
     if (Q.epi_scale != nullptr) return launch_igemm_impl<BN, false, false, false, true>(tm, tm, Q, st);
   }
-  if (Q.epi_scale != nullptr || Q.bst_y != nullptr) {
-    set_error("conv: the BN-backward moments epilogue needs a TMA-fed A operand; the folded-BN one a non-stem fprop");
+  if (Q.epi_scale != nullptr || Q.bst_y != nullptr || Q.in_scale != nullptr) {
+    set_error("conv: the BN-backward moments epilogue and the BN applied on load need a TMA-fed A operand; the folded-BN "
+              "epilogue a non-stem fprop");
     return DIRB200_ERR_ARG;
   }
   return launch_igemm_impl<BN, WGRAD, STEM>(tm, tm, Q, st);
@@ -860,11 +977,13 @@
 }
 
 static int conv_fprop_impl(const __nv_bfloat16* x, const __nv_bfloat16* w, __nv_bfloat16* y, const ConvShape& s, bool stem,
-                           cudaStream_t st, float* stat_partial, const ConvEpilogue* epi);
+                           cudaStream_t st, float* stat_partial, const ConvEpilogue* epi, const ConvInputBn* in_bn);
+
+bool conv_applies_input_bn(const ConvShape& s) { return is_plain_gemm(s, false) || im2col_enabled(); }
 
 int conv_fprop(const __nv_bfloat16* x, const __nv_bfloat16* w, __nv_bfloat16* y, const ConvShape& s, bool stem,
-               cudaStream_t st, float* stat_partial, StatLayout* layout) {
-  const int rc = conv_fprop_impl(x, w, y, s, stem, st, stat_partial, nullptr);
+               cudaStream_t st, float* stat_partial, StatLayout* layout, const ConvInputBn* in_bn) {
+  const int rc = conv_fprop_impl(x, w, y, s, stem, st, stat_partial, nullptr, in_bn);
   if (layout) *layout = t_last_layout;
   return rc;
 }
@@ -872,12 +991,14 @@
 int conv_fprop_affine(const __nv_bfloat16* x, const __nv_bfloat16* w, __nv_bfloat16* out, const ConvShape& s,
                       const ConvEpilogue& epi, cudaStream_t st) {
   DIRB_CHECK_ARG(epi.scale && epi.shift, "conv_fprop_affine: scale / shift missing");
-  return conv_fprop_impl(x, w, out, s, false, st, nullptr, &epi);
+  return conv_fprop_impl(x, w, out, s, false, st, nullptr, &epi, nullptr);
 }
 
 static int conv_fprop_impl(const __nv_bfloat16* x, const __nv_bfloat16* w, __nv_bfloat16* y, const ConvShape& s, bool stem,
-                           cudaStream_t st, float* stat_partial, const ConvEpilogue* epi) {
+                           cudaStream_t st, float* stat_partial, const ConvEpilogue* epi, const ConvInputBn* in_bn) {
   if (int rc = check_shape(s, stem, "conv_fprop")) return rc;
+  DIRB_CHECK_ARG(!in_bn || (!stem && conv_applies_input_bn(s) && in_bn->scale && in_bn->shift),
+                 "conv_fprop: the input BatchNorm is applied on load by TMA-fed GEMMs only");
   const int ktot = s.kh * s.kw * s.cin;
   IgemmParams P{};
   P.src = x; P.n = s.n; P.hs = s.h; P.ws = s.w; P.cs = s.cin; P.hm = s.ho; P.wm = s.wo;
@@ -892,6 +1013,9 @@
   P.stat_out = stat_partial;
   if (epi) {
     P.epi_scale = epi->scale; P.epi_shift = epi->shift; P.epi_res = epi->residual; P.epi_relu = epi->relu ? 1 : 0;
+  }
+  if (in_bn) {
+    P.in_scale = in_bn->scale; P.in_shift = in_bn->shift;
   }
   const int m_tiles = static_cast<int>((P.pixels + BM - 1) / BM);
   const int bn = pick_bn(s.cout);
@@ -1044,8 +1168,10 @@
 }
 
 int conv_wgrad_partials(const __nv_bfloat16* x, const __nv_bfloat16* dy, float* partial, const ConvShape& s, bool stem,
-                        int* splits_out, cudaStream_t st) {
+                        int* splits_out, cudaStream_t st, const ConvInputBn* in_bn) {
   if (int rc = check_shape(s, stem, "conv_wgrad")) return rc;
+  DIRB_CHECK_ARG(!in_bn || (!stem && conv_applies_input_bn(s) && in_bn->scale && in_bn->shift),
+                 "conv_wgrad: the input BatchNorm is applied on load by TMA-fed GEMMs only");
   IgemmParams P{};
   P.src = x; P.n = s.n; P.hs = s.h; P.ws = s.w; P.cs = s.cin; P.hm = s.ho; P.wm = s.wo;
   P.kh = s.kh; P.kw = s.kw; P.stride = s.stride; P.pad = s.pad; P.transposed = 0;
@@ -1059,6 +1185,9 @@
   const int splits = conv_wgrad_splits(s);
   P.kblocks_per_split = (P.num_kblocks + splits - 1) / splits;
   P.ldc = s.cout; P.out = partial;
+  if (in_bn) {
+    P.in_scale = in_bn->scale; P.in_shift = in_bn->shift;
+  }
   const int bn = wgrad_bn(s);
   P.n_tiles = s.cout / bn;
   const int m_tiles = (P.total_chunks + 1) / 2;
diff --git a/imbalanced-regression_b200/csrc/resnet_runner.cu b/imbalanced-regression_b200/csrc/resnet_runner.cu
--- a/imbalanced-regression_b200/csrc/resnet_runner.cu
+++ b/imbalanced-regression_b200/csrc/resnet_runner.cu
@@ -271,13 +271,25 @@
   return on;
 }
 
+static bool fused_apply() {
+  static const bool on = [] {
+    const char* e = getenv("DIRB200_FUSED_APPLY");
+    return e != nullptr && e[0] == '1';
+  }();
+  return on;
+}
+static bool reads_raw_input(const ConvLayer& next) { return fused_apply() && conv_applies_input_bn(next.s); }
+
 static int conv_bn_forward(dirb200_net* net, ConvLayer& cv, const __nv_bfloat16* in, const float* params,
-                           float* running, bool training, cudaStream_t st) {
+                           float* running, bool training, cudaStream_t st, const BNLayer* in_bn = nullptr,
+                           bool store_act = true) {
   BNLayer& bn = cv.bn;
   if (training) {
     StatLayout lay{};
     const bool fused = fused_stats();
-    RUNP(kFprop, conv_fprop(in, cv.wf, cv.y, cv.s, cv.stem, st, fused ? net->stat_partial : nullptr, &lay));
+    const ConvInputBn ib{in_bn ? in_bn->scale : nullptr, in_bn ? in_bn->shift : nullptr};
+    RUNP(kFprop, conv_fprop(in, cv.wf, cv.y, cv.s, cv.stem, st, fused ? net->stat_partial : nullptr, &lay,
+                            in_bn ? &ib : nullptr));
     if (!fused) {
       int nblk = 0;
       RUNP(kBnStats, bn_stats(cv.y, cv.rows, bn.c, net->stat_partial, &nblk, st));
@@ -291,14 +303,16 @@
     RUNP(kBnStats, bn_eval_coeffs(bn.c, params + bn.gamma_off, params + bn.beta_off, 1e-5f, running + bn.rm_off,
                                   running + bn.rv_off, bn.scale, bn.shift, st));
   }
-  if (cv.a)
+  if (cv.a && store_act)
     RUNP(kBnApply, bn_apply(cv.y, bn.scale, bn.shift, nullptr, nullptr, nullptr, nullptr, true, cv.rows, bn.c, cv.a, nullptr, st));
   return DIRB200_OK;
 }
 
-static int wgrad_step(dirb200_net* net, const __nv_bfloat16* x, const __nv_bfloat16* dy, ConvLayer& cv, cudaStream_t st) {
+static int wgrad_step(dirb200_net* net, const __nv_bfloat16* x, const __nv_bfloat16* dy, ConvLayer& cv, cudaStream_t st,
+                      const BNLayer* in_bn = nullptr) {
   int splits = 1;
-  RUNP(kWgrad, conv_wgrad_partials(x, dy, cv.wpart, cv.s, cv.stem, &splits, st));
+  const ConvInputBn ib{in_bn ? in_bn->scale : nullptr, in_bn ? in_bn->shift : nullptr};
+  RUNP(kWgrad, conv_wgrad_partials(x, dy, cv.wpart, cv.s, cv.stem, &splits, st, in_bn ? &ib : nullptr));
   return DIRB200_OK;
 }
 
@@ -360,9 +374,10 @@
   RUNP(kPool, bn_relu_maxpool_fwd(net->stem.y, net->stem.bn.scale, net->stem.bn.shift, net->n, net->stem.s.ho,
                                   net->stem.s.wo, 64, net->pool_out, net->pool_idx, st));
   for (Block& B : net->blocks) {
-    RUN(conv_bn_forward(net, B.c1, B.in, params, running, tr, st));
-    RUN(conv_bn_forward(net, B.c2, B.c1.a, params, running, tr, st));
-    RUN(conv_bn_forward(net, B.c3, B.c2.a, params, running, tr, st));
+    const bool raw2 = tr && reads_raw_input(B.c2), raw3 = tr && reads_raw_input(B.c3);
+    RUN(conv_bn_forward(net, B.c1, B.in, params, running, tr, st, nullptr, !raw2));
+    RUN(conv_bn_forward(net, B.c2, raw2 ? B.c1.y : B.c1.a, params, running, tr, st, raw2 ? &B.c1.bn : nullptr, !raw3));
+    RUN(conv_bn_forward(net, B.c3, raw3 ? B.c2.y : B.c2.a, params, running, tr, st, raw3 ? &B.c2.bn : nullptr));
     if (B.has_ds) {
       RUN(conv_bn_forward(net, B.ds, B.in, params, running, tr, st));
       RUNP(kBnApply, bn_apply(B.c3.y, B.c3.bn.scale, B.c3.bn.shift, nullptr, B.ds.y, B.ds.bn.scale, B.ds.bn.shift, true,
@@ -610,12 +625,13 @@
       RUNP(kBnBwdApply, bn_bwd_apply(nB, nullptr, B.c3.y, b3.coef, nullptr, nullptr, nullptr, nullptr, nullptr, B.c3.rows,
                                      b3.c, t1, nullptr, nullptr, st));
     gB_h = gB_w = 0;
-    RUN(wgrad_step(net, B.c2.a, t1, B.c3, st));
+    const bool raw3 = reads_raw_input(B.c3), raw2 = reads_raw_input(B.c2);
+    RUN(wgrad_step(net, raw3 ? B.c2.y : B.c2.a, t1, B.c3, st, raw3 ? &B.c2.bn : nullptr));
     StatLayout mlay{};
     bool mfused = false;
     RUN(dgrad_with_bn_moments(net, t1, B.c3, B.c2, t3, &mlay, &mfused, st));
     RUN(conv_bn_backward(net, B.c2, t3, params, grads, t1, st, mfused ? &mlay : nullptr));
-    RUN(wgrad_step(net, B.c1.a, t1, B.c2, st));
+    RUN(wgrad_step(net, raw2 ? B.c1.y : B.c1.a, t1, B.c2, st, raw2 ? &B.c1.bn : nullptr));
     RUN(dgrad_with_bn_moments(net, t1, B.c2, B.c1, t3, &mlay, &mfused, st));
     RUN(conv_bn_backward(net, B.c1, t3, params, grads, t1, st, mfused ? &mlay : nullptr));
     RUN(wgrad_step(net, B.in, t1, B.c1, st));
@@ -788,6 +804,16 @@
       default: DIRB_CHECK_ARG(false, "resnet_peek: bad selector %d", which);
     }
   }
+  if (act && block >= 0 && net->forward_was_training) {
+    const Block& B = net->blocks[block];
+    if (reads_raw_input(which == 1 ? B.c2 : B.c3)) {
+      const BNLayer& bn = cv->bn;
+      if (int rc = bn_apply(cv->y, bn.scale, bn.shift, nullptr, nullptr, nullptr, nullptr, true, cv->rows, bn.c, cv->a,
+                            nullptr, nullptr))
+        return rc;
+      DIRB_CUDA(cudaStreamSynchronize(nullptr));
+    }
+  }
   *ptr = act ? cv->a : cv->y;
   *rows = cv->rows;
   *channels = cv->s.cout;
diff --git a/imbalanced-regression_b200/csrc/tc.cuh b/imbalanced-regression_b200/csrc/tc.cuh
--- a/imbalanced-regression_b200/csrc/tc.cuh
+++ b/imbalanced-regression_b200/csrc/tc.cuh
@@ -118,6 +118,28 @@
       : DIRB_F16(0), DIRB_F16(16), DIRB_F16(32), DIRB_F16(48)
       : "l"(adesc), "l"(bdesc), "r"(accumulate), "n"(TA), "n"(TB));
 }
+template <int TB>
+__device__ __forceinline__ void wgmma_m64n64_rs(float (&d)[32], const uint32_t* a, uint64_t bdesc, uint32_t accumulate) {
+  asm volatile(
+      "{\n.reg .pred p;\nsetp.ne.b32 p, %37, 0;\n"
+      "wgmma.mma_async.sync.aligned.m64n64k16.f32.bf16.bf16 {"
+      DIRB_R8(0, 1, 2, 3, 4, 5, 6, 7) DIRB_R8(8, 9, 10, 11, 12, 13, 14, 15) DIRB_R8(16, 17, 18, 19, 20, 21, 22, 23)
+      "%24, %25, %26, %27, %28, %29, %30, %31}, {%32, %33, %34, %35}, %36, p, 1, 1, %38;\n}\n"
+      : DIRB_F16(0), DIRB_F16(16)
+      : "r"(a[0]), "r"(a[1]), "r"(a[2]), "r"(a[3]), "l"(bdesc), "r"(accumulate), "n"(TB));
+}
+template <int TB>
+__device__ __forceinline__ void wgmma_m64n128_rs(float (&d)[64], const uint32_t* a, uint64_t bdesc, uint32_t accumulate) {
+  asm volatile(
+      "{\n.reg .pred p;\nsetp.ne.b32 p, %69, 0;\n"
+      "wgmma.mma_async.sync.aligned.m64n128k16.f32.bf16.bf16 {"
+      DIRB_R8(0, 1, 2, 3, 4, 5, 6, 7) DIRB_R8(8, 9, 10, 11, 12, 13, 14, 15) DIRB_R8(16, 17, 18, 19, 20, 21, 22, 23)
+      DIRB_R8(24, 25, 26, 27, 28, 29, 30, 31) DIRB_R8(32, 33, 34, 35, 36, 37, 38, 39) DIRB_R8(40, 41, 42, 43, 44, 45, 46, 47)
+      DIRB_R8(48, 49, 50, 51, 52, 53, 54, 55)
+      "%56, %57, %58, %59, %60, %61, %62, %63}, {%64, %65, %66, %67}, %68, p, 1, 1, %70;\n}\n"
+      : DIRB_F16(0), DIRB_F16(16), DIRB_F16(32), DIRB_F16(48)
+      : "r"(a[0]), "r"(a[1]), "r"(a[2]), "r"(a[3]), "l"(bdesc), "r"(accumulate), "n"(TB));
+}
 #undef DIRB_R8
 #undef DIRB_F16
 #undef DIRB_F4
@@ -125,6 +147,20 @@
 __device__ __forceinline__ void wgmma_bf16(float (&d)[BN / 2], uint64_t adesc, uint64_t bdesc, uint32_t accumulate) {
   if constexpr (BN == 128) wgmma_m64n128<TA, TB>(d, adesc, bdesc, accumulate);
   else wgmma_m64n64<TA, TB>(d, adesc, bdesc, accumulate);
+}
+template <int BN, int TB>
+__device__ __forceinline__ void wgmma_bf16_rs(float (&d)[BN / 2], const uint32_t* a, uint64_t bdesc, uint32_t accumulate) {
+  if constexpr (BN == 128) wgmma_m64n128_rs<TB>(d, a, bdesc, accumulate);
+  else wgmma_m64n64_rs<TB>(d, a, bdesc, accumulate);
+}
+
+__device__ __forceinline__ void ldmatrix_x4(uint32_t* r, uint32_t addr) {
+  asm volatile("ldmatrix.sync.aligned.m8n8.x4.shared.b16 {%0, %1, %2, %3}, [%4];"
+               : "=r"(r[0]), "=r"(r[1]), "=r"(r[2]), "=r"(r[3]) : "r"(addr) : "memory");
+}
+__device__ __forceinline__ void ldmatrix_x4_trans(uint32_t* r, uint32_t addr) {
+  asm volatile("ldmatrix.sync.aligned.m8n8.x4.trans.shared.b16 {%0, %1, %2, %3}, [%4];"
+               : "=r"(r[0]), "=r"(r[1]), "=r"(r[2]), "=r"(r[3]) : "r"(addr) : "memory");
 }
 
 __device__ __forceinline__ uint64_t make_smem_desc(uint32_t saddr, uint32_t lbo_bytes, uint32_t sbo_bytes) {
diff --git a/include/dirb200.h b/include/dirb200.h
--- a/include/dirb200.h
+++ b/include/dirb200.h
@@ -160,6 +160,12 @@
 int dirb200_conv_dgrad_bn_moments(const void* dy, const void* w_dgrad, void* dx, int n, int h, int w, int cin, int cout,
                                   int kh, int kw, int stride, int pad, const void* y_prev, const float* scale,
                                   const float* shift, float* partial, int* layout_host, void* stream);
+int dirb200_conv_fprop_apply(const void* y_prev, const float* scale, const float* shift, const void* w_fprop, void* y,
+                             int n, int h, int w, int cin, int cout, int kh, int kw, int stride, int pad, float* partial,
+                             int* layout_host, void* stream);
+int dirb200_conv_wgrad_apply(const void* y_prev, const float* scale, const float* shift, const void* dy, float* dw,
+                             void* workspace, size_t workspace_bytes, int n, int h, int w, int cin, int cout, int kh,
+                             int kw, int stride, int pad, int accumulate, void* stream);
 int dirb200_bn_finalize_layout(const float* partial, const int* layout_host, int64_t rows, int c, const float* gamma,
                                const float* beta, float eps, float momentum, float* running_mean, float* running_var,
                                float* mean_out, float* invstd_out, float* scale_out, float* shift_out, void* stream);
```

Result: no change. 7681, median of 6 (-0.0%).
